# eriq-augustine/KB2E

Measured on AMD Instinct MI355X. Metric: training triples/sec (1/2/4/8 MI355X) + FB15k Hits@10(Filter), higher is better.
Workload: dtype f64

## Files before the change

kb2e_amd/csrc/engine.hip:

```cpp
#include <hip/hip_runtime.h>
#include <hip/hip_ext.h>
#include <hipcub/hipcub.hpp>

#include <algorithm>
#include <cmath>
#include <cstdio>
#include <cstring>
#include <map>
#include <memory>
#include <stdexcept>
#include <string>
#include <vector>

#include "../../include/kb2e_engine.h"
#include "glibc_rand.hpp"
#include "hip_util.hpp"
#include "eval.hpp"
#include "predict.hpp"
#include "host_data.hpp"
#include "kernels_common.hpp"
#include "kernels_index.hpp"
#include "kernels_transe.hpp"
#include "kernels_transe_long.hpp"
#include "kernels_relowner.hpp"
#include "kernels_sampler.hpp"
#include "kernels_parallel.hpp"
#include "kernels_transr_parallel.hpp"
#include "kernels_transr_mfma.hpp"
#include "transr_cons.hpp"
#include "kernels_transh_parallel.hpp"
#include "textio.hpp"

using namespace kb2e;

namespace {

constexpr int kGlibcBlock = 4096;

int bits_for(int64_t v) {
    int b = 1;
    while ((1ll << b) <= v) ++b;
    return b;
}

struct Timer {
    double ms = 0;
    int64_t launches = 0;
};

}

struct kb2e_ctx;
struct MergeState;
void merge_free(MergeState* m);
namespace {
void setup_relowner_buffers(kb2e_ctx* c);
template <typename T>
void run_batch_relowner(kb2e_ctx* c, int64_t b);
void check_dataflow(kb2e_ctx* c);
void build_owner_index(kb2e_ctx* c);
void prepare_relowner_kernels();
void setup_transr_parallel(kb2e_ctx* c);
void build_transr_tiles(kb2e_ctx* c, bool tiles, hipStream_t st, int set);
template <typename T>
void run_batch_transr_parallel(kb2e_ctx* c, int64_t b);
template <typename T, int CH>
void run_batch_transh_parallel(kb2e_ctx* c, int64_t b);
}

struct kb2e_ctx {
    int64_t device_bytes = 0;
    kb2e_config cfg{};
    std::string err;
    GlibcRand rng{1};
    TripleStore ts;
    DevBuf rel_order;
    bool have_triples = false, have_params = false;
    int tables_read = 0;
    int n = 0, ld = 0, ch = 1, nw = 2, esize = 8;
    int64_t B = 0, nb = 0, S = 0;
    int32_t sub = 1;
    int64_t Bs = 0, nbi = 0;
    DevBuf snap_ent, snap_rel, snap_w;
    DevBuf sb_x, sb_d, sb_y, sb_wpart, sb_rpart, sb_pflag, sb_cons_tile, sb_cpairs, sb_vio, sb_cnrows;
    hipStream_t suba_stream = nullptr;
    hipEvent_t ev_adone[2] = {nullptr, nullptr}, ev_bdone[2] = {nullptr, nullptr};
    uint64_t wait_ticks = 0;
    hipStream_t stream = nullptr;

    DevBuf ent, rel, w;
    int64_t w_elems = 0;
    DevBuf heads, tails, rels;
    DevBuf si_[2], sj_[2], side_[2];
    int cur = 0;
    int32_t* pin_si = nullptr;
    int32_t* pin_sj = nullptr;
    uint8_t* pin_side = nullptr;
    hipStream_t side_stream = nullptr;
    DevBuf words, levels, jfin, sidefin, filter_slots, filter_bloom, pr_dev, consumed_dev;
    DevBuf trip;
    int32_t trip_eb = 0, trip_rb = 0;
    DevBuf glibc_pow;
    DevBuf chain_table, chain_super, chain_sc, chain_ch, chain_overflow;
    bool sampler_doubling = false;
    int64_t* pin_consumed = nullptr;
    uint32_t* pin_win = nullptr;
    DevBuf raw_words, glibc_starts, glibc_table, win_dev;
    int64_t nraw = 0, nraw_cap = 0;
    int levels_cap = 0;
    double words_per_sample = 6.0;
    bool prefetch_valid = false;
    uint64_t rng_version = 0, prefetch_version = 0;
    int64_t prefetch_gen = 0, committed_gen = -1, index_pre_gen = -2;
    bool next_pending = false;
    hipEvent_t ev_index = nullptr;
    hipEvent_t ev_sampled = nullptr, ev_epoch_done = nullptr;
    bool host_sampler = false;
    std::vector<int32_t> rp_si, rp_sj;
    std::vector<uint8_t> rp_side;
    int64_t rp_pos = 0;
    KeyLayout kl{};
    int slots = 6;
    DevBuf keys, keys_sorted, sort_tmp, flags, idx, seg_start, nseg, nvalid, batch_seg;
    size_t sort_tmp_bytes = 0, scan_tmp_bytes = 0;
    DevBuf act, loss;
    DevBuf xbits, xreal;
    DevBuf aux, aux2;
    RelOwnerPlan plan;
    DevBuf owner, tickets, ent_done, wsnap, transr_work, transr_work_alt, owner_seg, dataflow_err, wtouched, desc, cdesc, ocount;
    int num_cus = 256;
    uint32_t batch_stamp = 0;
    uint32_t rpar_ptab_mask = 0;
    int32_t gram_min = 48;
    int32_t long_min = 192;
    int32_t apply_long_min = 256;
    int32_t par_long_cap = 1, apply_grid = 256;
    DevBuf par_long_list, par_long_count;
    DevBuf hpar_orth;
    DevBuf hpar_ids;
    DevBuf hpar_tag;
    uint32_t hpar_stamp = 0;
    DevBuf hpar_clk;
    DevBuf hpar_count;
    uint32_t hpar_orth_min = 0;
    int32_t hpar_orth_q = 0;
    DevBuf ev_iota, ev_slot_sorted, ev_inv, seg_row, ev_meta, ev_words;
    int32_t rpar_St = 8, rpar_max_tiles = 1, rpar_tile_threads = 256, rpar_tgroup = 1;
    bool rpar_no_constraint = false;
    bool rpar_mfma = false;
    bool rpar_cons_wave = false;
    size_t rpar_cons_lds = 0;
    bool rpar_cons_seq = false;
    size_t rpar_seq_lds = 0;
    DevBuf rpar_vio;
    bool rpar_cons_wide = false;
    size_t rpar_wide_lds = 0;
    bool rpar_cons_gen = false;
    size_t rpar_gen_lds = 0;
    bool rpar_widep = false;
    WideGeom rpar_wg;
    DevBuf rpar_wsc;
    DevBuf rpar_pflag, rpar_cons_tile, rpar_cpairs, rpar_cnrows;
    DevBuf rpar_y, rpar_wpart, rpar_rpart, rpar_tile_act, rpar_pair, rpar_relpair, rpar_relpair_stamp, rpar_scan_pre, rpar_tiles,
        rpar_ntiles, rpar_tile_first, rpar_rel_begin, rpar_scan;
    DevBuf rpar_ptab;
    DevBuf rpar_batch_t0, rpar_td_r, rpar_td_cnt, rpar_td_kk, rpar_td_ent;
    DevBuf sh_rpar_batch_t0, sh_rpar_td_r, sh_rpar_td_cnt, sh_rpar_td_kk, sh_rpar_td_ent;
    DevBuf rpar_brel, sh_rpar_brel, rpar_bnrel, sh_rpar_bnrel;
    int64_t rpar_brel_cap = 0;
    int32_t* pin_bnrel = nullptr;
    int32_t* pin_sh_bnrel = nullptr;
    hipStream_t fold_stream = nullptr;
    hipEvent_t ev_fold_a = nullptr, ev_fold_b = nullptr;
    DevBuf long_list, long_count;
    DevBuf sh_keys, sh_keys_sorted, sh_sort_tmp, sh_flags, sh_idx, sh_seg_start, sh_nseg, sh_nvalid, sh_batch_seg,
        sh_ev_slot_sorted, sh_ev_inv, sh_seg_row, sh_rpar_ntiles, sh_rpar_rel_begin, sh_rpar_tile_first,
        sh_rpar_tiles, sh_par_long_list, sh_par_long_count;
    DevBuf stats;
    double acc_loss = 0;
    int64_t acc_active = 0;
    int64_t reduced_upto = 0;
    int64_t epoch_pos = 0;
    bool epoch_ready = false;
    bool prof = false;
    int32_t prof_period = 1;
    int64_t prof_counter = 0;
    bool prof_batch = true;
    std::map<std::string, Timer> timers;
    struct Pending {
        std::string name;
        hipEvent_t a, b;
    };
    std::vector<Pending> pending;
    std::vector<hipEvent_t> event_pool;
    MergeState* mg = nullptr;

    ~kb2e_ctx() {
        if (mg) merge_free(mg);
        if (pin_si) (void)hipHostFree(pin_si);
        if (pin_sj) (void)hipHostFree(pin_sj);
        if (pin_side) (void)hipHostFree(pin_side);
        if (pin_win) (void)hipHostFree(pin_win);
        if (pin_consumed) (void)hipHostFree(pin_consumed);
        if (pin_bnrel) (void)hipHostFree(pin_bnrel);
        if (pin_sh_bnrel) (void)hipHostFree(pin_sh_bnrel);
        flush_timers();
        if (ev_sampled) (void)hipEventDestroy(ev_sampled);
        if (ev_epoch_done) (void)hipEventDestroy(ev_epoch_done);
        if (ev_index) (void)hipEventDestroy(ev_index);
        if (side_stream) (void)hipStreamDestroy(side_stream);
        if (suba_stream) (void)hipStreamDestroy(suba_stream);
        for (hipEvent_t e : {ev_adone[0], ev_adone[1], ev_bdone[0], ev_bdone[1]})
            if (e) (void)hipEventDestroy(e);
        if (fold_stream) (void)hipStreamDestroy(fold_stream);
        if (ev_fold_a) (void)hipEventDestroy(ev_fold_a);
        if (ev_fold_b) (void)hipEventDestroy(ev_fold_b);
        for (auto e : event_pool) (void)hipEventDestroy(e);
        if (stream) (void)hipStreamDestroy(stream);
    }

    bool f64() const { return cfg.precision == 64; }
    bool parallel() const { return cfg.schedule == KB2E_SCHEDULE_PARALLEL; }
    int32_t* si() const { return si_[cur].as<int32_t>(); }
    int32_t* sj() const { return sj_[cur].as<int32_t>(); }
    uint8_t* side() const { return side_[cur].as<uint8_t>(); }

    hipEvent_t get_event() {
        if (!event_pool.empty()) {
            hipEvent_t e = event_pool.back();
            event_pool.pop_back();
            return e;
        }
        hipEvent_t e;
        HIPCHK(hipEventCreate(&e));
        return e;
    }

    template <class F>
    void timed(const char* name, F&& f) {
        timed_on(stream, name, f);
    }
    hipEvent_t begin_span() {
        if (!prof || !prof_batch) return nullptr;
        hipEvent_t a = get_event();
        HIPCHK(hipEventRecord(a, stream));
        return a;
    }
    void end_span(const char* name, hipEvent_t a) {
        if (!a) return;
        hipEvent_t b = get_event();
        HIPCHK(hipEventRecord(b, stream));
        pending.push_back({name, a, b});
    }
    template <class F>
    void timed_on(hipStream_t st, const char* name, F&& f) {
        if (!prof || !prof_batch) {
            f();
            return;
        }
        hipEvent_t a = get_event(), b = get_event();
        HIPCHK(hipEventRecord(a, st));
        f();
        HIPCHK(hipEventRecord(b, st));
        pending.push_back({name, a, b});
        if (pending.size() > 4096) flush_timers();
    }

    hipEvent_t span_a = nullptr;
    const char* span_name = nullptr;
    void ev_begin(const char* name, hipEvent_t& a) {
        a = nullptr;
        if (!prof || !prof_batch) return;
        a = span_a = get_event();
        span_name = name;
    }
    void ev_end(hipEvent_t& b) {
        b = nullptr;
        if (!span_a) return;
        b = get_event();
        pending.push_back({span_name, span_a, b});
        span_a = nullptr;
    }
    template <typename... KArgs, typename... Args>
    void launch(void (*kernel)(KArgs...), dim3 grid, dim3 block, size_t lds, hipEvent_t a, hipEvent_t b,
                Args... args) {
        if (a || b) hipExtLaunchKernelGGL(kernel, grid, block, lds, stream, a, b, 0, args...);
        else hipLaunchKernelGGL(kernel, grid, block, lds, stream, args...);
        HIPCHK(hipGetLastError());
    }

    void flush_timers() {
        if (pending.empty()) return;
        (void)hipStreamSynchronize(stream);
        for (auto& p : pending) {
            float ms = 0;
            if (hipEventElapsedTime(&ms, p.a, p.b) == hipSuccess) {
                timers[p.name].ms += ms;
                timers[p.name].launches += 1;
            }
            event_pool.push_back(p.a);
            event_pool.push_back(p.b);
        }
        pending.clear();
    }
};

namespace {

kb2e_status fail(kb2e_ctx* c, kb2e_status s, const std::string& msg) {
    if (c) c->err = msg;
    return s;
}

struct TallyScope {
    int64_t* prev;
    explicit TallyScope(int64_t* t) : prev(DevBuf::tally_now) { DevBuf::tally_now = t; }
    ~TallyScope() { DevBuf::tally_now = prev; }
};

template <class F>
kb2e_status guarded(kb2e_ctx* c, F&& f) {
    if (!c) return KB2E_EINVAL;
    TallyScope ts(&c->device_bytes);
    try {
        return f();
    } catch (const HipError& e) {
        return fail(c, KB2E_EDEVICE, e.what());
    } catch (const Unsupported& e) {
        return fail(c, KB2E_EUNSUPPORTED, e.what());
    } catch (const std::invalid_argument& e) {
        return fail(c, KB2E_EINVAL, e.what());
    } catch (const std::bad_alloc&) {
        return fail(c, KB2E_ENOMEM, "host out of memory");
    } catch (const std::exception& e) {
        return fail(c, KB2E_EDEVICE, e.what());
    }
}


template <typename T>
void upload_rows(kb2e_ctx* c, DevBuf& dst, const double* src, int64_t rows, int n, int ld) {
    std::vector<T> tmp((size_t)rows * ld, T(0));
    for (int64_t r = 0; r < rows; ++r)
        for (int i = 0; i < n; ++i) tmp[(size_t)r * ld + i] = (T)src[(size_t)r * n + i];
    HIPCHK(hipMemcpyAsync(dst.p, tmp.data(), tmp.size() * sizeof(T), hipMemcpyHostToDevice, c->stream));
    HIPCHK(hipStreamSynchronize(c->stream));
}

template <typename T>
void download_rows(kb2e_ctx* c, const DevBuf& src, double* dst, int64_t rows, int n, int ld) {
    std::vector<T> tmp((size_t)rows * ld);
    HIPCHK(hipMemcpyAsync(tmp.data(), src.p, tmp.size() * sizeof(T), hipMemcpyDeviceToHost, c->stream));
    HIPCHK(hipStreamSynchronize(c->stream));
    for (int64_t r = 0; r < rows; ++r)
        for (int i = 0; i < n; ++i) dst[(size_t)r * n + i] = (double)tmp[(size_t)r * ld + i];
}

int64_t w_rows(const kb2e_ctx* c) {
    if (c->cfg.model == KB2E_TRANSH) return c->cfg.num_relations;
    if (c->cfg.model == KB2E_TRANSR) return (int64_t)c->cfg.num_relations * c->n;
    return 0;
}

void sync_wsnap(kb2e_ctx* c) {
    if (c->cfg.model != KB2E_TRANSR) return;
    HIPCHK(hipMemcpyAsync(c->wsnap.p, c->w.p, c->w.bytes, hipMemcpyDeviceToDevice, c->stream));
    HIPCHK(hipStreamSynchronize(c->stream));
}

void upload_tables(kb2e_ctx* c, const double* e, const double* r, const double* w) {
    const int64_t ne = c->cfg.num_entities, nr = c->cfg.num_relations;
    if (c->f64()) {
        if (e) upload_rows<double>(c, c->ent, e, ne, c->n, c->ld);
        if (r) upload_rows<double>(c, c->rel, r, nr, c->n, c->ld);
        if (w && w_rows(c)) upload_rows<double>(c, c->w, w, w_rows(c), c->n, c->ld);
    } else {
        if (e) upload_rows<float>(c, c->ent, e, ne, c->n, c->ld);
        if (r) upload_rows<float>(c, c->rel, r, nr, c->n, c->ld);
        if (w && w_rows(c)) upload_rows<float>(c, c->w, w, w_rows(c), c->n, c->ld);
    }
    if (w) sync_wsnap(c);
}


std::vector<std::pair<DevBuf*, DevBuf*>> index_bufs(kb2e_ctx* c) {
    return {{&c->keys, &c->sh_keys}, {&c->keys_sorted, &c->sh_keys_sorted}, {&c->sort_tmp, &c->sh_sort_tmp},
            {&c->flags, &c->sh_flags}, {&c->idx, &c->sh_idx}, {&c->seg_start, &c->sh_seg_start},
            {&c->nseg, &c->sh_nseg}, {&c->nvalid, &c->sh_nvalid}, {&c->batch_seg, &c->sh_batch_seg},
            {&c->ev_slot_sorted, &c->sh_ev_slot_sorted}, {&c->ev_inv, &c->sh_ev_inv}, {&c->seg_row, &c->sh_seg_row},
            {&c->rpar_ntiles, &c->sh_rpar_ntiles}, {&c->rpar_rel_begin, &c->sh_rpar_rel_begin},
            {&c->rpar_tile_first, &c->sh_rpar_tile_first}, {&c->rpar_tiles, &c->sh_rpar_tiles},
            {&c->rpar_batch_t0, &c->sh_rpar_batch_t0}, {&c->rpar_td_r, &c->sh_rpar_td_r},
            {&c->rpar_td_cnt, &c->sh_rpar_td_cnt}, {&c->rpar_td_kk, &c->sh_rpar_td_kk},
            {&c->rpar_td_ent, &c->sh_rpar_td_ent}, {&c->rpar_brel, &c->sh_rpar_brel},
            {&c->rpar_bnrel, &c->sh_rpar_bnrel},

            {&c->par_long_list, &c->sh_par_long_list}, {&c->par_long_count, &c->sh_par_long_count}};
}

void swap_index(kb2e_ctx* c) {
    for (auto& pr : index_bufs(c)) {
        std::swap(pr.first->p, pr.second->p);
        std::swap(pr.first->bytes, pr.second->bytes);
    }
    std::swap(c->pin_bnrel, c->pin_sh_bnrel);
}

void alloc_shadow_index(kb2e_ctx* c) {
    for (auto& pr : index_bufs(c)) {
        pr.second->free();
        if (pr.first->p) pr.second->alloc(pr.first->bytes);
    }
    c->index_pre_gen = -2;
}

void build_index(kb2e_ctx* c, hipStream_t st, int set) {
    const int64_t nkeys = c->S * c->slots;
    KeyArgs ka{};
    ka.heads = c->heads.as<int32_t>();
    ka.tails = c->tails.as<int32_t>();
    ka.rels = c->rels.as<int32_t>();
    ka.si = c->si_[set].as<int32_t>();
    ka.sj = c->sj_[set].as<int32_t>();
    ka.side = c->side_[set].as<uint8_t>();
    ka.owner = c->cfg.model == KB2E_TRANSE ? nullptr : c->owner.as<int32_t>();
    ka.nsamples = c->S;
    ka.B = (int32_t)c->B;
    ka.sub = c->sub;
    ka.Bs = (int32_t)c->Bs;
    ka.ne = c->cfg.num_entities;
    ka.kl = c->kl;
    ka.keys = c->keys.as<uint64_t>();
    const int grid = (int)((c->S + 255) / 256);
    auto build = [&] {
        if (c->cfg.model == KB2E_TRANSR)
            emit_keys_kernel<8, true><<<grid, 256, 0, st>>>(ka);
        else
            emit_keys_kernel<6, false><<<grid, 256, 0, st>>>(ka);
        HIPCHK(hipGetLastError());
        const int lo_bit = getenv("KB2E_SORT_FULLKEY") ? 0 : c->kl.row_shift();
        size_t tb = c->sort_tmp_bytes;
        if (c->parallel() && c->cfg.model != KB2E_TRANSR) {
            HIPCHK(hipcub::DeviceRadixSort::SortPairs(c->sort_tmp.p, tb, c->keys.as<uint64_t>(),
                                                      c->keys_sorted.as<uint64_t>(), c->ev_iota.as<int32_t>(),
                                                      c->ev_slot_sorted.as<int32_t>(), (int)nkeys, lo_bit,
                                                      c->kl.total_bits(), st));
            inverse_perm_kernel<<<(int)((nkeys + 255) / 256), 256, 0, st>>>(c->ev_slot_sorted.as<int32_t>(),
                                                                                  nkeys, c->ev_inv.as<int32_t>());
            HIPCHK(hipGetLastError());
        } else {
            HIPCHK(hipcub::DeviceRadixSort::SortKeys(c->sort_tmp.p, tb, c->keys.as<uint64_t>(),
                                                     c->keys_sorted.as<uint64_t>(), (int)nkeys, lo_bit,
                                                     c->kl.total_bits(), st));
        }
        const int g2 = (int)((nkeys + 255) / 256);
        seg_flags_kernel<<<g2, 256, 0, st>>>(c->keys_sorted.as<uint64_t>(), nkeys, c->kl,
                                                     c->flags.as<int32_t>(), c->nvalid.as<int32_t>());
        HIPCHK(hipGetLastError());
        tb = c->sort_tmp_bytes;
        HIPCHK(hipcub::DeviceScan::ExclusiveSum(c->sort_tmp.p, tb, c->flags.as<int32_t>(),
                                                c->idx.as<int32_t>(), (int)nkeys, st));
        seg_scatter_kernel<<<g2, 256, 0, st>>>(c->flags.as<int32_t>(), c->idx.as<int32_t>(), nkeys,
                                                       c->seg_start.as<int32_t>(), c->nseg.as<int32_t>(),
                                                       c->nvalid.as<int32_t>());
        HIPCHK(hipGetLastError());
        batch_begin_kernel<<<256, 256, 0, st>>>(c->keys_sorted.as<uint64_t>(), c->seg_start.as<int32_t>(),
                                                        c->nseg.as<int32_t>(), (int)c->nbi, c->kl,
                                                        c->batch_seg.as<int32_t>());
// ... 1439 lines not shown
```

kb2e_amd/csrc/engine_transr_parallel.inc:

```
namespace {

constexpr int32_t kRParLongMin = 128;

template <typename T, bool P, bool G>
const void* tile_fn(int nb) {
    switch (nb) {
        case 1: return (const void*)transr_tile_mfma_kernel<T, P, G, 1>;
        case 2: return (const void*)transr_tile_mfma_kernel<T, P, G, 2>;
        case 3: return (const void*)transr_tile_mfma_kernel<T, P, G, 3>;
        case 4: return (const void*)transr_tile_mfma_kernel<T, P, G, 4>;
        case 5: return (const void*)transr_tile_mfma_kernel<T, P, G, 5>;
        case 6: return (const void*)transr_tile_mfma_kernel<T, P, G, 6>;
        case 7: return (const void*)transr_tile_mfma_kernel<T, P, G, 7>;
        case 8: return (const void*)transr_tile_mfma_kernel<T, P, G, 8>;
    }
    throw std::runtime_error("TransR tile kernel: n > 128");
}

template <typename T>
const void* cons_tile_fn(int nb) {
    switch (nb) {
        case 1: return (const void*)transr_cons_tile_kernel<T, 1>;
        case 2: return (const void*)transr_cons_tile_kernel<T, 2>;
        case 3: return (const void*)transr_cons_tile_kernel<T, 3>;
        case 4: return (const void*)transr_cons_tile_kernel<T, 4>;
        case 5: return (const void*)transr_cons_tile_kernel<T, 5>;
        case 6: return (const void*)transr_cons_tile_kernel<T, 6>;
        case 7: return (const void*)transr_cons_tile_kernel<T, 7>;
        case 8: return (const void*)transr_cons_tile_kernel<T, 8>;
    }
    throw std::runtime_error("transRNorm tile kernel: n > 128");
}

template <typename T>
size_t rpar_lds(const kb2e_ctx* c) {
    return rpar_tile_lds<T>(c->n, c->ld, c->rpar_St);
}

template <typename T>
size_t rmfma_lds(const kb2e_ctx* c, bool cons) {
    return cons ? rmfma_cons_lds<T>(c->n, c->rpar_St) : rmfma_tile_lds<T>(c->n, c->rpar_St);
}

size_t rpar_scan_lds(const kb2e_ctx* c) {
    return (size_t)kScanChunk * 2 * c->n * 8 + (size_t)std::max(1, 1024 / (2 * c->n)) * 2 * c->n * 8;
}

int choose_mfma_samples(int n, int esize, bool tile_only = false) {
    const char* tk = getenv("KB2E_RPAR_TILE_KB");
    const size_t tile_kb = tk ? (size_t)std::max(16, std::min(160, atoi(tk))) : 96;
    for (int St = 8; St >= 1; St >>= 1) {
        const size_t a = esize == 8 ? rmfma_tile_lds<double>(n, St) : rmfma_tile_lds<float>(n, St);
        const size_t b = tile_only ? 0 : esize == 8 ? rmfma_cons_lds<double>(n, St) : rmfma_cons_lds<float>(n, St);
        if (std::max(a, b) <= (tile_only ? tile_kb : 150) * 1024) return St;
    }
    return 0;
}

int choose_tile_samples(int n, int ld, int esize) {
    const size_t budget = (size_t)n * ld * esize > 40 * 1024 ? 150 * 1024 : 64 * 1024;
    for (int St = 32; St > 1; St >>= 1) {
        const size_t b = esize == 8 ? rpar_tile_lds<double>(n, ld, St) : rpar_tile_lds<float>(n, ld, St);
        if (b <= budget) return St;
    }
    return 1;
}

void setup_transr_parallel(kb2e_ctx* c) {
    const kb2e_config& g = c->cfg;
    const size_t es = (size_t)c->esize;
    const char* ck0 = getenv("KB2E_RPAR_CONS");
    const bool wide_planned = c->f64() && c->n > 64 && cons_chainw_supported(c->n) &&
                              !(ck0 && (std::string(ck0) == "jacobi" || std::string(ck0) == "tile"));
    c->rpar_widep = wide_par_supported(c->n);
    const int mst = c->rpar_widep ? 0 : choose_mfma_samples(c->n, c->esize, wide_planned);
    const char* mf = getenv("KB2E_RPAR_MFMA");
    c->rpar_mfma = mst > 0 && !(mf && mf[0] == '0');
    if (c->rpar_widep) c->rpar_wg = wide_setup(c->n, c->ld, c->esize);
    c->rpar_St = c->rpar_widep ? c->rpar_wg.St : c->rpar_mfma ? mst : choose_tile_samples(c->n, c->ld, c->esize);
    if (const char* nc = getenv("KB2E_RPAR_NOC")) c->rpar_no_constraint = nc[0] == '1';
    c->rpar_tile_threads = wide_planned && c->rpar_mfma ? 512 : 256;
    if (const char* tt = getenv("KB2E_RPAR_TILE_THREADS")) c->rpar_tile_threads = atoi(tt) >= 512 ? 512 : 256;
    c->rpar_tgroup = c->rpar_tile_threads == 512 ? 8 : 1;
    if (const char* tg = getenv("KB2E_RPAR_TGROUP")) c->rpar_tgroup = std::max(1, std::min(kTileGroupMax, atoi(tg)));
    if (const char* st = getenv("KB2E_RPAR_ST")) c->rpar_St = std::max(1, std::min(c->rpar_St, atoi(st)));
    if (c->rpar_mfma && 4 * c->rpar_St + 1 > 64) throw std::runtime_error("transRNorm tile: St > 15");
    c->rpar_max_tiles = (int)(std::min<int64_t>(g.num_relations, c->B) + c->B / c->rpar_St + 1);
    const int64_t nkeys = c->S * c->slots;
    c->rpar_y.alloc((size_t)c->B * 2 * c->ld * es);
    const bool cw = cons_wave_supported(c->n) && mst > 0;
    c->rpar_wpart.alloc((size_t)c->rpar_max_tiles * (cw ? kConsPpt : 1) * c->n * c->ld * es);
    c->rpar_rpart.alloc((size_t)c->rpar_max_tiles * c->ld * es);
    c->rpar_tile_act.alloc((size_t)(nkeys + 1) * 4);
    c->rpar_pair.alloc((size_t)c->B * 4 * c->ld * es);
    c->rpar_relpair.alloc((size_t)g.num_relations * c->ld * es);
    c->rpar_relpair_stamp.alloc((size_t)g.num_relations * 4);
    memset_sync(c->rpar_relpair_stamp.p, 0, c->rpar_relpair_stamp.bytes);
    c->rpar_tiles.alloc((size_t)(nkeys + 1) * sizeof(RTile));
    c->rpar_ntiles.alloc((size_t)(nkeys + 1) * 4);
    c->rpar_tile_first.alloc((size_t)(nkeys + 1) * 4);
    c->rpar_rel_begin.alloc((size_t)c->nbi * 4);
    c->rpar_brel_cap = std::min<int64_t>(g.num_relations, c->Bs);
    c->rpar_brel.alloc((size_t)c->nbi * c->rpar_brel_cap * 4);
    c->rpar_bnrel.alloc((size_t)c->nbi * 4);
    for (int32_t** h : {&c->pin_bnrel, &c->pin_sh_bnrel}) {
        if (*h) (void)hipHostFree(*h);
        *h = nullptr;
        HIPCHK(hipHostMalloc((void**)h, (size_t)c->nbi * 4, 0));
        std::memset(*h, 0, (size_t)c->nbi * 4);
    }
    if (c->rpar_widep) c->rpar_wsc.alloc((size_t)c->rpar_brel_cap * c->n * c->ld * 8);
    else c->rpar_wsc.free();
    if (c->sub > 1) {
        c->snap_ent.alloc(c->ent.bytes);
        c->snap_rel.alloc(c->rel.bytes);
        c->snap_w.alloc(c->w.bytes);
        for (DevBuf* d : {&c->snap_ent, &c->snap_rel, &c->snap_w}) memset_sync(d->p, 0, d->bytes);
        if (!c->suba_stream) {
            int lo = 0, hi = 0;
            HIPCHK(hipDeviceGetStreamPriorityRange(&lo, &hi));
            HIPCHK(hipStreamCreateWithPriority(&c->suba_stream, hipStreamNonBlocking, hi));
            for (hipEvent_t* e : {&c->ev_adone[0], &c->ev_adone[1], &c->ev_bdone[0], &c->ev_bdone[1]})
                HIPCHK(hipEventCreateWithFlags(e, hipEventDisableTiming));
        }
    } else {
        for (DevBuf* d : {&c->snap_ent, &c->snap_rel, &c->snap_w}) d->free();
    }
    if (g.num_entities >= (1 << kPtabEntBits) - 1 || g.num_relations >= (1 << kPtabRelBits) - 1 ||
        c->B * 4 >= (1 << kPtabSlotBits))
        throw std::invalid_argument("PARALLEL TransR: at most 2^24 - 2 entities, 2^18 - 2 relations, 2^20 - 1 samples a batch");
    {
        size_t sz = 1024;
        while (sz < (size_t)c->B * 4 * 3) sz <<= 1;
        c->rpar_ptab_mask = (uint32_t)(sz - 1);
        c->rpar_ptab.alloc(3 * sz * 8);
        memset_sync(c->rpar_ptab.p, 0xff, 3 * sz * 8);
    }
    const int scan_chunk = c->rpar_widep ? c->rpar_wg.chunk : kScanChunk;
    c->rpar_scan.alloc((size_t)((2 * c->B + scan_chunk - 1) / scan_chunk) * 2 * c->n * 8);
    c->rpar_scan_pre.alloc(c->rpar_scan.bytes);
    c->rpar_pflag.alloc((size_t)c->B * 4);
    c->rpar_cons_tile.alloc((size_t)c->rpar_max_tiles * (cw ? kConsPpt : 1) * 4);
    if (cw) {
        c->rpar_cpairs.alloc((size_t)c->rpar_max_tiles * 2 * kCPairs * 4);
        c->rpar_vio.alloc((size_t)c->rpar_max_tiles * kCPairs * 4);
        c->rpar_cnrows.alloc((size_t)c->rpar_max_tiles * 4);
    }
    size_t tb = 0;
    HIPCHK(hipcub::DeviceScan::ExclusiveSum(nullptr, tb, (int32_t*)nullptr, (int32_t*)nullptr, (int)(nkeys + 1),
                                            c->stream));
    if (tb > c->sort_tmp_bytes) {
        c->sort_tmp_bytes = tb;
        c->sort_tmp.alloc(tb);
    }
    const size_t lds = c->f64() ? rpar_lds<double>(c) : rpar_lds<float>(c);
    auto allow = [&](const void* k) {
        (void)hipFuncSetAttribute(k, hipFuncAttributeMaxDynamicSharedMemorySize, (int)lds);
    };
    allow((const void*)transr_tile_kernel<double, true, true>);
    allow((const void*)transr_tile_kernel<double, true, false>);
    allow((const void*)transr_tile_kernel<double, false, true>);
    allow((const void*)transr_tile_kernel<float, true, true>);
    allow((const void*)transr_tile_kernel<float, true, false>);
    allow((const void*)transr_tile_kernel<float, false, true>);
    allow((const void*)transr_constraint_kernel<double>);
    allow((const void*)transr_constraint_kernel<float>);
    c->rpar_cons_wave = false;
    if (c->rpar_mfma) {
        const size_t l1 = c->f64() ? rmfma_lds<double>(c, false) : rmfma_lds<float>(c, false);
        const size_t l2 = c->f64() ? rmfma_lds<double>(c, true) : rmfma_lds<float>(c, true);
        const int nb = rm_np(c->n) / 16;
        for (const void* k : {tile_fn<double, true, true>(nb), tile_fn<double, true, false>(nb),
                              tile_fn<double, false, true>(nb), tile_fn<float, true, true>(nb),
                              tile_fn<float, true, false>(nb), tile_fn<float, false, true>(nb)})
            (void)hipFuncSetAttribute(k, hipFuncAttributeMaxDynamicSharedMemorySize, (int)l1);
        if (!wide_planned)
            for (int nb = 1; nb <= 8; ++nb)
                (void)hipFuncSetAttribute(c->f64() ? cons_tile_fn<double>(nb) : cons_tile_fn<float>(nb),
                                          hipFuncAttributeMaxDynamicSharedMemorySize, (int)l2);
        const char* ck = getenv("KB2E_RPAR_CONS");
        c->rpar_cons_wave = cw && c->rpar_St <= 8 && !(ck && std::string(ck) == "tile");
        if (c->rpar_cons_wave) c->rpar_cons_lds = cons_wave_setup(c->n, c->rpar_St, c->esize);
        c->rpar_cons_seq = c->rpar_cons_wave && c->f64() && !(ck && std::string(ck) == "jacobi");
        if (c->rpar_cons_seq) {
            c->rpar_seq_lds = cons_seq_setup(c->n);
        }
    }
    {
        const char* ck = getenv("KB2E_RPAR_CONS");
        const bool jac = ck && (std::string(ck) == "jacobi" || std::string(ck) == "tile");
        const char* chn = getenv("KB2E_RPAR_CHAIN");
        c->rpar_cons_wide = !c->rpar_cons_seq && c->f64() && cons_chainw_supported(c->n) && !jac;
        if (c->rpar_cons_wide) c->rpar_wide_lds = cons_chainw_setup(c->n);
        const bool force_gen = chn && std::string(chn) == "gen";
        if (force_gen && !jac) c->rpar_cons_seq = c->rpar_cons_wide = false;
        c->rpar_cons_gen = !c->rpar_cons_seq && !c->rpar_cons_wide && !jac && cons_chaing_supported(c->n);
        if (c->rpar_cons_gen) c->rpar_gen_lds = cons_chaing_setup(c->n, c->esize);
        if (c->rpar_widep) c->rpar_cons_seq = c->rpar_cons_wide = c->rpar_cons_gen = false;
        if (!c->rpar_cons_seq && !c->rpar_cons_wide && !c->rpar_cons_gen && !c->rpar_widep && !c->rpar_no_constraint &&
            !jac)
            throw Unsupported("PARALLEL TransR: no pair-by-pair transRNorm at this width");
    }
    if (c->rpar_cons_wave || c->rpar_mfma) {
        const size_t nt = (size_t)c->nbi * c->rpar_max_tiles + 1;
        c->rpar_batch_t0.alloc((size_t)(c->nbi + 1) * 4);
        c->rpar_td_r.alloc(nt * 4);
        c->rpar_td_cnt.alloc(nt * 4);
        c->rpar_td_kk.alloc(nt * 8 * 4);
        c->rpar_td_ent.alloc(nt * 32 * 4);
    } else {
        for (DevBuf* d : {&c->rpar_batch_t0, &c->rpar_td_r, &c->rpar_td_cnt, &c->rpar_td_kk, &c->rpar_td_ent}) d->free();
    }
    {
        const std::pair<DevBuf*, DevBuf*> sets[] = {
            {&c->sb_x, &c->xreal}, {&c->sb_d, &c->aux}, {&c->sb_y, &c->rpar_y}, {&c->sb_wpart, &c->rpar_wpart},
            {&c->sb_rpart, &c->rpar_rpart}, {&c->sb_pflag, &c->rpar_pflag}, {&c->sb_cons_tile, &c->rpar_cons_tile},
            {&c->sb_cpairs, &c->rpar_cpairs}, {&c->sb_vio, &c->rpar_vio}, {&c->sb_cnrows, &c->rpar_cnrows}};
        for (const auto& pr : sets) {
            pr.first->free();
            if (c->sub > 1 && pr.second->p) {
                pr.first->alloc(pr.second->bytes);
                memset_sync(pr.first->p, 0, pr.first->bytes);
            }
        }
    }
    for (const void* k : {(const void*)rpar_scan_energy_kernel<double>, (const void*)rpar_scan_energy_kernel<float>})
        (void)hipFuncSetAttribute(k, hipFuncAttributeMaxDynamicSharedMemorySize, (int)rpar_scan_lds(c));
    (void)hipGetLastError();
}

void build_transr_tiles(kb2e_ctx* c, bool tiles, hipStream_t st, int set) {
    const int64_t nkeys = c->S * c->slots;
    rtile_count_kernel<<<1024, 256, 0, st>>>(c->keys_sorted.as<uint64_t>(), c->seg_start.as<int32_t>(),
                                                    c->nseg.as<int32_t>(), nkeys + 1, c->kl, c->cfg.num_entities,
                                                    c->rpar_St, c->rpar_ntiles.as<int32_t>(),
                                                    c->rpar_rel_begin.as<int32_t>());
    HIPCHK(hipGetLastError());
    if (!tiles) return;
    size_t tb = c->sort_tmp_bytes;
    HIPCHK(hipcub::DeviceScan::ExclusiveSum(c->sort_tmp.p, tb, c->rpar_ntiles.as<int32_t>(),
                                            c->rpar_tile_first.as<int32_t>(), (int)(nkeys + 1), st));
    rtile_scatter_kernel<<<1024, 256, 0, st>>>(c->rpar_ntiles.as<int32_t>(), c->rpar_tile_first.as<int32_t>(),
                                                      c->nseg.as<int32_t>(), c->rpar_tiles.as<RTile>());
    HIPCHK(hipGetLastError());
    if (c->rpar_brel.p) {
        rel_list_kernel<<<(int)c->nbi, 1024, 0, st>>>(c->rpar_rel_begin.as<int32_t>(), c->batch_seg.as<int32_t>(),
                                                     c->seg_row.as<int32_t>(), c->cfg.num_entities,
                                                     c->rel_order.as<int32_t>(), c->cfg.num_relations,
                                                     c->rpar_brel_cap, c->rpar_brel.as<int32_t>(),
                                                     c->rpar_bnrel.as<int32_t>());
        HIPCHK(hipGetLastError());
        HIPCHK(hipMemcpyAsync(c->pin_bnrel, c->rpar_bnrel.p, (size_t)c->nbi * 4, hipMemcpyDeviceToHost, st));
    }
    if (c->rpar_td_r.p) {
        RTileDescArgs d{};
        d.keys = c->keys_sorted.as<uint64_t>();
        d.seg_start = c->seg_start.as<int32_t>();
        d.seg_row = c->seg_row.as<int32_t>();
        d.tiles = c->rpar_tiles.as<RTile>();
        d.tile_first = c->rpar_tile_first.as<int32_t>();
        d.nseg = c->nseg.as<int32_t>();
        d.batch_seg = c->batch_seg.as<int32_t>();
        d.nb = (int32_t)c->nbi;
        d.sub = c->sub;
        d.Bs = (int32_t)c->Bs;
        d.St = c->rpar_St;
        d.ne = c->cfg.num_entities;
        d.B = (int32_t)c->B;
        d.kl = c->kl;
        d.si = c->si_[set].as<int32_t>();
        d.sj = c->sj_[set].as<int32_t>();
        d.side = c->side_[set].as<uint8_t>();
        d.heads = c->heads.as<int32_t>();
        d.tails = c->tails.as<int32_t>();
        d.batch_t0 = c->rpar_batch_t0.as<int32_t>();
        d.td_r = c->rpar_td_r.as<int32_t>();
        d.td_cnt = c->rpar_td_cnt.as<int32_t>();
        d.td_kk = c->rpar_td_kk.as<int32_t>();
        d.td_ent = c->rpar_td_ent.as<int32_t>();
        rtile_desc_kernel<<<2048, 256, 0, st>>>(d);
        HIPCHK(hipGetLastError());
    }
}

DevBuf& buf_set(int set, DevBuf& s0, DevBuf& s1) { return set ? s1 : s0; }

bool sub_overlap_on() {
    const char* e = getenv("KB2E_SUB_OVERLAP");
    return !(e && e[0] == '0');
}

template <typename T>
void run_subbatch_transr_parallel(kb2e_ctx* c, int64_t b, int j) {
    const bool ov = c->sub > 1 && sub_overlap_on();
    const bool side = ov && j > 0;
    const int set = ov ? (j & 1) : 0;
    hipStream_t sa = side ? c->suba_stream : c->stream;
    const int64_t ib = b * c->sub + j;
    const int64_t first = b * c->B + (int64_t)j * c->Bs;
    const int64_t cnt = std::min<int64_t>(c->Bs, c->B - (int64_t)j * c->Bs);
    RParArgs a{};
    a.heads = c->heads.as<int32_t>();
    a.tails = c->tails.as<int32_t>();
    a.rels = c->rels.as<int32_t>();
    a.si = c->si() + first;
    a.sj = c->sj() + first;
    a.side = c->side() + first;
    a.B = (int32_t)cnt;
    a.n = c->n;
    a.ld = c->ld;
    a.ne = c->cfg.num_entities;
    a.nr = c->cfg.num_relations;
    a.St = c->rpar_St;
    a.tgroup = c->rpar_tgroup;
    a.batch = (int32_t)ib;
    a.lr = c->cfg.learning_rate;
    a.margin = c->cfg.margin;
    a.compat = c->cfg.transr_compat;
    a.l1 = c->cfg.distance == 0;
    a.keys = c->keys_sorted.as<uint64_t>();
    a.seg_start = c->seg_start.as<int32_t>();
    a.batch_seg = c->batch_seg.as<int32_t>();
    a.seg_row = c->seg_row.as<int32_t>();
    a.rel_begin = c->rpar_rel_begin.as<int32_t>();
    a.tile_first = c->rpar_tile_first.as<int32_t>();
    a.tiles = c->rpar_tiles.as<RTile>();
    a.kl = c->kl;
    a.act = c->act.as<uint8_t>() + first;
    a.loss = c->loss.as<double>() + first;
    a.proj = c->aux2.as<double>();
    a.tile_act = c->rpar_tile_act.as<int32_t>();
    a.batch_t0 = c->rpar_batch_t0.as<int32_t>();
    a.td_r = c->rpar_td_r.as<int32_t>();
    a.td_cnt = c->rpar_td_cnt.as<int32_t>();
    a.td_kk = c->rpar_td_kk.as<int32_t>();
    a.td_ent = c->rpar_td_ent.as<int32_t>();
    a.brel = c->rpar_brel.as<int32_t>() + ib * c->rpar_brel_cap;
    a.nrel = c->pin_bnrel[ib];
    if (a.nrel < 1 || a.nrel > c->rpar_brel_cap) throw std::logic_error("batch relation count out of range");
    {
        unsigned long long* t0 = c->rpar_ptab.as<unsigned long long>();
        const size_t sz = (size_t)c->rpar_ptab_mask + 1;
        a.ptab = t0 + (c->batch_stamp % 3) * sz;
        a.ptab_next = t0 + ((c->batch_stamp + 1) % 3) * sz;
        a.ptab_mask = c->rpar_ptab_mask;
    }
    RParBufs<T> bf{};
    bf.ent = c->ent.as<T>();
    bf.rel = c->rel.as<T>();
    bf.W = c->w.as<T>();
    bf.x = buf_set(set, c->xreal, c->sb_x).as<T>();
    bf.d = buf_set(set, c->aux, c->sb_d).as<T>();
    bf.y = buf_set(set, c->rpar_y, c->sb_y).as<T>();
    bf.wpart = buf_set(set, c->rpar_wpart, c->sb_wpart).as<T>();
    bf.rpart = buf_set(set, c->rpar_rpart, c->sb_rpart).as<T>();
    bf.pair = c->rpar_pair.as<T>();
    bf.relpair = c->rpar_relpair.as<T>();
    bf.relpair_stamp = c->rpar_relpair_stamp.as<uint32_t>();
    bf.stamp = ++c->batch_stamp;
    bf.err = c->dataflow_err.as<uint32_t>() + 1;
    if (c->rpar_mfma) {
        bf.pflag = buf_set(set, c->rpar_pflag, c->sb_pflag).as<uint8_t>();
        bf.cons_tile = buf_set(set, c->rpar_cons_tile, c->sb_cons_tile).as<int32_t>();
        bf.cons_ppt = c->rpar_cons_wave ? kConsPpt : 1;
        bf.cpairs = buf_set(set, c->rpar_cpairs, c->sb_cpairs).as<int32_t>();
        bf.vio = buf_set(set, c->rpar_vio, c->sb_vio).as<int32_t>();
        bf.cnrows = buf_set(set, c->rpar_cnrows, c->sb_cnrows).as<int32_t>();
        bf.stats = getenv("KB2E_RPAR_STATS") != nullptr;
        bf.last_renorm = c->rpar_cons_seq ? 1 : 0;
        if (const char* dbg = getenv("KB2E_CONS_DBG")) bf.dbg = atoi(dbg);
        if (const char* cl = getenv("KB2E_RPAR_CHAIN_LIST")) bf.chain_list = std::max(64, atoi(cl));
        if (const char* ct = getenv("KB2E_RPAR_CHAIN_TILES")) bf.chain_tiles = std::max(1, atoi(ct));
        if (const char* rc = getenv("KB2E_RPAR_REC_CAP")) bf.rec_cap = std::max(4, atoi(rc));
    }
    if (c->rpar_cons_wide || c->rpar_cons_gen || c->rpar_widep) {
        bf.pflag = buf_set(set, c->rpar_pflag, c->sb_pflag).as<uint8_t>();
        if (const char* dbg = getenv("KB2E_CONS_DBG")) bf.dbg = atoi(dbg);
        bf.stats = getenv("KB2E_RPAR_STATS") != nullptr;
        bf.last_renorm = 1;
    }
    RParBufs<T> bfa = bf;
    if (c->sub > 1) {
        bfa.ent = c->snap_ent.as<T>();
        bfa.rel = c->snap_rel.as<T>();
        bfa.W = c->snap_w.as<T>();
    }
    if (side && j == 1) HIPCHK(hipStreamWaitEvent(sa, c->ev_adone[0], 0));
    if (side && j >= 2) HIPCHK(hipStreamWaitEvent(sa, c->ev_bdone[set], 0));
    auto a_done = [&] {
        if (!ov) return;
        HIPCHK(hipEventRecord(c->ev_adone[set], sa));
        if (side) HIPCHK(hipStreamWaitEvent(c->stream, c->ev_adone[set], 0));
    };
    auto b_done = [&] {
        if (ov) HIPCHK(hipEventRecord(c->ev_bdone[set], c->stream));
    };
    if (c->rpar_widep) {
        c->timed_on(sa, "score", [&] {
            wide_phase_a<T>(a, bfa, c->rpar_wg, c->rpar_max_tiles, c->rpar_scan.as<double>(),
                            c->rpar_scan_pre.as<double>(), c->transr_work.as<double>(),
                            c->transr_work_alt.as<double>(), sa);
        });
        if (c->cfg.transr_compat) std::swap(c->transr_work.p, c->transr_work_alt.p);
        a_done();
        c->timed("apply", [&] {
            wide_phase_b<T>(a, bf, c->rpar_wg, c->rpar_wsc.as<double>(), !c->rpar_no_constraint,
                            (int)std::min<int64_t>(c->cfg.num_relations, c->Bs), c->stream);
        });
        b_done();
        if (c->pending.size() > 4096) c->flush_timers();
        return;
    }
    const size_t lds = rpar_lds<T>(c);
    const int tgrid = c->rpar_max_tiles;
    const int rel_waves = (int)std::min<int64_t>(c->cfg.num_relations, c->B) * (c->n + 1);
    const int rgrid = (rel_waves + 3) / 4;
    const int egrid = 256;
    const bool mf = c->rpar_mfma;
    const size_t lt = mf ? rmfma_lds<T>(c, false) : lds;
    const size_t lc = mf ? rmfma_lds<T>(c, true) : lds;
    const int tb = mf ? c->rpar_tile_threads : 256;
    auto tile = [&](auto proj, auto grad) {
        constexpr bool P = decltype(proj)::value, G = decltype(grad)::value;
        if (mf) {
            void* args[] = {&a, &bfa};
            int pt = tb;
            if (P && !G) {
                pt = 256;
                if (const char* e = getenv("KB2E_RPAR_PROJ_THREADS")) pt = atoi(e) >= 512 ? 512 : 256;
            }
            HIPCHK(hipLaunchKernel(tile_fn<T, P, G>(rm_np(c->n) / 16), dim3(tgrid), dim3(pt), args,
                                   rmfma_tile_lds<T>(c->n, c->rpar_St, P, G), sa));
        } else {
            transr_tile_kernel<T, P, G><<<tgrid, tb, lt, sa>>>(a, bfa);
        }
        HIPCHK(hipGetLastError());
    };
    using yes = std::true_type;
    using no = std::false_type;
    auto pair_first = [&] {
        if (c->rpar_no_constraint) return;
        transr_pair_first_kernel<<<(int)((4 * c->B + 255) / 256), 256, 0, sa>>>(a);
        HIPCHK(hipGetLastError());
    };
    c->timed_on(sa, "score", [&] {
        if (c->cfg.transr_compat) {
            if (c->rpar_cons_wave) proj_wave_launch<T>(a, bfa, tgrid, sa);
            else tile(yes(), no());
            const int64_t calls = 2 * (int64_t)a.B;
            const int nchunks = (int)((calls + kScanChunk - 1) / kScanChunk);
            rpar_scan_sums_kernel<<<nchunks, 256, 0, sa>>>(a.proj, calls, c->ld, c->n,
                                                                  c->rpar_scan.as<double>());
            const char* sp = getenv("KB2E_RPAR_SCAN_PREFIX");
            const bool use_pre = sp ? sp[0] == '1' : nchunks > kScanDirectMax;
            double* pre = nullptr;
            if (use_pre) {
                pre = c->rpar_scan_pre.as<double>();
                rpar_scan_prefix_kernel<<<(2 * c->n + 31) / 32, 1024, 0, sa>>>(
                    c->rpar_scan.as<double>(), nchunks, 2 * c->n, c->transr_work.as<double>(), pre);
            }
            rpar_scan_energy_kernel<T><<<nchunks, 1024, rpar_scan_lds(c), sa>>>(
                a, bfa, c->rpar_scan.as<double>(), nchunks, c->transr_work.as<double>(),
                c->transr_work_alt.as<double>(), pre);
            HIPCHK(hipGetLastError());
            std::swap(c->transr_work.p, c->transr_work_alt.p);
            if (c->rpar_cons_wave) grad_wave_launch<T>(a, bfa, tgrid, sa);
            else tile(no(), yes());
        } else if (c->rpar_cons_wave) {
            proj_wave_launch<T>(a, bfa, tgrid, sa);
            grad_wave_launch<T>(a, bfa, tgrid, sa);
        } else {
            tile(yes(), yes());
            pair_first();
        }
    });
    a_done();
    hipEvent_t e0, e1;
    c->ev_begin("apply", e0);
    const char* fz = getenv("KB2E_RPAR_FUSE");
    const bool fuse = !(fz && fz[0] == '0');
    const char* r8 = getenv("KB2E_RPAR_ROWS8");
    const int rmode = c->n <= 64 ? 4 : (c->n <= 128 && r8 && r8[0] == '1') ? 8 : 0;
    const bool rows4 = rmode != 0;
    const int rel_waves4 = (int)std::min<int64_t>(c->cfg.num_relations, c->B) * ((c->n + 4) / 4);
    const int rw = rows4 ? rel_waves4 : rel_waves;
    const int fgrid = egrid + (rw + 15) / 16;
    auto rows_fn = [&](auto pass1) {
        constexpr bool P = decltype(pass1)::value;
        return rmode == 4 ? transr_rows_kernel<T, P, 4> : rmode == 8 ? transr_rows_kernel<T, P, 8>
                                                                     : transr_rows_kernel<T, P, 0>;
    };
    using yes1 = std::true_type;
    if (c->rpar_no_constraint) {
        c->ev_end(e1);
        c->launch(rows_fn(yes1()), dim3(fgrid), dim3(1024), 0, e0, e1, a, bf, kRParLongMin, egrid);
        b_done();
        return;
    }
    if (fuse) {
        c->launch(rows_fn(yes1()), dim3(fgrid), dim3(1024), 0, e0, nullptr, a, bf, kRParLongMin, egrid);
    } else {
        c->launch(transr_rel_rows_kernel<T, true>, dim3(rgrid), dim3(256), 0, e0, nullptr, a, bf);
        transr_entity_kernel<T, true><<<egrid, 1024, 0, c->stream>>>(a, bf, kRParLongMin);
        HIPCHK(hipGetLastError());
    }
    if (mf && c->rpar_cons_seq) {
        if constexpr (std::is_same<T, double>::value) cons_seq_launch(a, bf, c->rpar_seq_lds, c->stream);
    } else if (c->rpar_cons_gen) {
        cons_chaing_launch<T>(a, bf, c->rpar_gen_lds, c->stream);
    } else if (c->rpar_cons_wide) {
        if constexpr (std::is_same<T, double>::value) cons_chainw_launch(a, bf, c->rpar_wide_lds, c->stream);
    } else if (mf && c->rpar_cons_wave) {
        cons_wave_launch<T>(a, bf, tgrid, c->rpar_cons_lds, c->stream);
    } else if (mf) {
        void* args[] = {&a, &bf};
        HIPCHK(hipLaunchKernel(cons_tile_fn<T>(rm_np(c->n) / 16), dim3(tgrid), dim3(512), args, lc, c->stream));
    } else {
        transr_constraint_kernel<T><<<tgrid, 256, lc, c->stream>>>(a, bf);
    }
    HIPCHK(hipGetLastError());
    c->ev_end(e1);
    const char* f2 = getenv("KB2E_RPAR_FUSE2");
    if (c->rpar_cons_seq || c->rpar_cons_wide || c->rpar_cons_gen) {
        c->launch(transr_entity_kernel<T, false>, dim3(egrid), dim3(1024), 0, nullptr, e1, a, bf, kRParLongMin);
    } else if (f2 && f2[0] == '1') {
        c->launch(rows_fn(std::false_type()), dim3(fgrid), dim3(1024), 0, nullptr, e1, a, bf, kRParLongMin, egrid);
    } else {
        if (rmode == 4) transr_rel_rows4_kernel<T, false, 4><<<(rel_waves4 + 3) / 4, 256, 0, c->stream>>>(a, bf);
        else if (rmode == 8) transr_rel_rows4_kernel<T, false, 8><<<(rel_waves4 + 3) / 4, 256, 0, c->stream>>>(a, bf);
        else transr_rel_rows_kernel<T, false><<<rgrid, 256, 0, c->stream>>>(a, bf);
        HIPCHK(hipGetLastError());
        c->launch(transr_entity_kernel<T, false>, dim3(egrid), dim3(1024), 0, nullptr, e1, a, bf, kRParLongMin);
    }
    b_done();
    if (c->pending.size() > 4096) c->flush_timers();
}

template <typename T>
void run_batch_transr_parallel(kb2e_ctx* c, int64_t b) {
    if (c->sub > 1) {
        for (auto pr : {std::make_pair(&c->snap_ent, &c->ent), std::make_pair(&c->snap_rel, &c->rel),
                        std::make_pair(&c->snap_w, &c->w)})
            HIPCHK(hipMemcpyAsync(pr.first->p, pr.second->p, pr.second->bytes, hipMemcpyDeviceToDevice, c->stream));
    }
    for (int j = 0; j < c->sub; ++j) run_subbatch_transr_parallel<T>(c, b, j);
}

}
```

kb2e_amd/csrc/kernels_transr_parallel.hpp:

```cpp
#pragma once

#include <type_traits>

#include "kernels_common.hpp"

namespace kb2e {

struct RTile {
    int32_t seg, q;
};

struct RParArgs {
    const int32_t* heads;
    const int32_t* tails;
    const int32_t* rels;
    const int32_t* si;
    const int32_t* sj;
    const uint8_t* side;
    int32_t B, n, ld, ne, nr, St;
    int32_t batch;
    int32_t tgroup;
    double lr, margin;
    int32_t compat, l1;
    const uint64_t* keys;
    const int32_t* seg_start;
    const int32_t* batch_seg;
    const int32_t* seg_row;
    const int32_t* rel_begin;
    const int32_t* tile_first;
    const RTile* tiles;
    KeyLayout kl;
    uint8_t* act;
    double* loss;
    double* proj;
    int32_t* tile_act;
    unsigned long long* ptab;
    unsigned long long* ptab_next;
    uint32_t ptab_mask;
    const int32_t* batch_t0;
    const int32_t* td_r;
    const int32_t* td_cnt;
    const int32_t* td_kk;
    const int32_t* td_ent;
    const int32_t* brel;
    int32_t nrel;
};

static __attribute__((unused)) __global__ __launch_bounds__(1024) void rel_list_kernel(
    const int32_t* rel_begin, const int32_t* batch_seg, const int32_t* seg_row, int32_t ne, const int32_t* rel_order,
    int32_t nr, int64_t cap, int32_t* brel, int32_t* nrel) {
    __shared__ int32_t wsum[16];
    const int b = blockIdx.x, t = threadIdx.x, w = t >> 6, l = t & 63;
    const int s0 = rel_begin[b], s1 = batch_seg[b + 1];
    int32_t* out = brel + (int64_t)b * cap;
    int total = 0;
    for (int base = 0; base < nr; base += 1024) {
        const int q = base + t;
        const int r = q < nr ? rel_order[q] : -1;
        bool here = false;
        if (r >= 0 && s0 < s1) {
            int lo = s0, hi = s1 - 1;
            const int want = ne + r;
            while (lo < hi) {
                const int mid = (lo + hi) >> 1;
                if (seg_row[mid] < want) lo = mid + 1;
                else hi = mid;
            }
            here = seg_row[lo] == want;
        }
        const uint64_t m = __ballot(here);
        if (l == 0) wsum[w] = __popcll(m);
        __syncthreads();
        int off = total;
        for (int k = 0; k < w; ++k) off += wsum[k];
        int all = 0;
        for (int k = 0; k < 16; ++k) all += wsum[k];
        if (here) out[off + __popcll(m & ((1ull << l) - 1))] = r;
        total += all;
        __syncthreads();
    }
    if (t == 0) nrel[b] = total;
}

constexpr int kPtabEntBits = 24, kPtabRelBits = 18, kPtabSlotBits = 22;
constexpr unsigned long long kPtabEmpty = ~0ull;

__device__ __forceinline__ unsigned long long ptab_key(int r, int e) {
    return ((unsigned long long)r << kPtabEntBits) | (unsigned long long)e;
}
__device__ __forceinline__ uint32_t ptab_hash(int r, int e) {
    return ((uint32_t)e * 2654435761u) ^ ((uint32_t)r * 0x9E3779B1u + 0x7F4A7C15u);
}

__device__ __forceinline__ void ptab_insert(const RParArgs& a, int r, int e, int slot) {
    const unsigned long long key = ptab_key(r, e);
    const unsigned long long word = (key << kPtabSlotBits) | (unsigned long long)slot;
    uint32_t h = ptab_hash(r, e) & a.ptab_mask;
    while (true) {
        const unsigned long long old = atomicCAS(a.ptab + h, kPtabEmpty, word);
        if (old == kPtabEmpty) return;
        if ((old >> kPtabSlotBits) == key) {
            atomicMin(a.ptab + h, word);
            return;
        }
        h = (h + 1) & a.ptab_mask;
    }
}

__device__ __forceinline__ int ptab_first(const RParArgs& a, int r, int e) {
    const unsigned long long key = ptab_key(r, e);
    uint32_t h = ptab_hash(r, e) & a.ptab_mask;
    while (true) {
        const unsigned long long w = a.ptab[h];
        if (w == kPtabEmpty) return -1;
        if ((w >> kPtabSlotBits) == key) return (int)(w & ((1ull << kPtabSlotBits) - 1));
        h = (h + 1) & a.ptab_mask;
    }
}

__device__ __forceinline__ void ptab_clear_next(const RParArgs& a, int64_t tid, int64_t nthreads) {
    for (int64_t q = tid; q <= (int64_t)a.ptab_mask; q += nthreads) a.ptab_next[q] = kPtabEmpty;
}

__device__ __forceinline__ bool transr_pair_dup(const RParArgs& a, int slot, int r, int e) {
    return ptab_first(a, r, e) < slot;
}
__device__ __forceinline__ bool transr_relpair_dup(const RParArgs& a, int r) {
    return ptab_first(a, r, r) >= 0;
}

static __attribute__((unused)) __global__ __launch_bounds__(256) void transr_pair_first_kernel(RParArgs a) {
    const int slot = blockIdx.x * blockDim.x + threadIdx.x;
    ptab_clear_next(a, slot, (int64_t)gridDim.x * blockDim.x);
    if (slot >= 4 * a.B) return;
    const int kk = slot >> 2, u = (slot >> 1) & 1, role = slot & 1;
    if (!a.act[kk]) return;
    const int i0 = a.si[kk], jj = a.sj[kk];
    const int h = a.heads[i0], tt = a.tails[i0];
    const int hh = u ? (a.side[kk] ? h : jj) : h;
    const int th = u ? (a.side[kk] ? jj : tt) : tt;
    ptab_insert(a, a.rels[i0], role ? th : hh, slot);
}

template <typename T>
struct RParBufs {
    T* ent;
    T* rel;
    T* W;
    T* x;
    T* d;
    T* y;
    T* wpart;
    T* rpart;
    T* pair;
    T* relpair;
    uint32_t* relpair_stamp;
    uint32_t stamp;
    uint8_t* pflag;
    int32_t* cons_tile;
    int32_t cons_ppt;
    int32_t* cpairs;
    int32_t* cnrows;
    int32_t stats;
    int32_t last_renorm;
    int32_t dbg;
    int32_t chain_list;
    int32_t chain_tiles;
    int32_t rec_cap;
    int32_t* vio;
    uint32_t* err;
};

__host__ __device__ constexpr int rm_up16_host_dev(int v) { return (v + 15) & ~15; }
constexpr int kCPairs = 64;

template <typename T>
__host__ __device__ constexpr int rpar_lds_w(int n, int ld) {
    return n * ld;
}

__device__ __forceinline__ void tile_range(const RParArgs& a, int t, int& r, int& e0, int& cnt) {
    const RTile tl = a.tiles[t];
    const int p0 = a.seg_start[tl.seg], p1 = a.seg_start[tl.seg + 1];
    r = a.seg_row[tl.seg] - a.ne;
    const int ns = (p1 - p0) / 2;
    const int f = tl.q * a.St;
    e0 = p0 + 2 * f;
    cnt = min(a.St, ns - f);
}

template <typename T>
__device__ __forceinline__ void stage_matrix(T* Wl, const T* Wg, int n, int ld) {
    for (int idx = threadIdx.x; idx < n * ld; idx += blockDim.x) Wl[idx] = Wg[idx];
}

template <typename T>
__device__ __forceinline__ void project4(const T* Wl, int ld, int n, const T* v4 , T (&p)[4][2]) {
    const int l = lane_id();
    const int i = 2 * l;
#pragma unroll
    for (int q = 0; q < 4; ++q) p[q][0] = p[q][1] = T(0);
    if (i >= n) return;
    for (int j = 0; j < n; ++j) {
        const T w0 = Wl[j * ld + i], w1 = Wl[j * ld + i + 1];
#pragma unroll
        for (int q = 0; q < 4; ++q) {
            const T vj = v4[q * ld + j];
            p[q][0] += w0 * vj;
            p[q][1] += w1 * vj;
        }
    }
}

template <typename T>
__device__ __forceinline__ void matvec_rows(const T* Wl, int ld, int n, const T* xl, T (&y)[2]) {
    const int l = lane_id();
    const int j = 2 * l;
    y[0] = y[1] = T(0);
    if (j >= n) return;
    const T* r0 = Wl + j * ld;
    const T* r1 = Wl + (j + 1) * ld;
    const bool has1 = j + 1 < n;
    for (int i = 0; i < n; ++i) {
        const T xi = xl[i];
        y[0] += r0[i] * xi;
        if (has1) y[1] += r1[i] * xi;
    }
}

template <typename T>
__device__ __forceinline__ void lane_pair_load(const T* row, int n, T (&v)[2]) {
    const int e = 2 * lane_id();
    v[0] = e < n ? row[e] : T(0);
    v[1] = e + 1 < n ? row[e + 1] : T(0);
}
template <typename T>
__device__ __forceinline__ void lane_pair_store(T* row, int n, const T (&v)[2]) {
    const int e = 2 * lane_id();
    if (e < n) row[e] = v[0];
    if (e + 1 < n) row[e + 1] = v[1];
}

template <typename T>
__device__ __forceinline__ void rank_sum_rows(const T* Dl, const T* Xl, int U, int ld, int n, int j, T (&acc)[2]) {
    const int i = 2 * lane_id();
    acc[0] = acc[1] = T(0);
    if (i >= n) return;
    for (int u = 0; u < U; ++u) {
        const T dj = Dl[u * ld + j];
        acc[0] += dj * Xl[u * ld + i];
        acc[1] += dj * Xl[u * ld + i + 1];
    }
}

template <typename T>
__host__ __device__ constexpr size_t rpar_tile_lds(int n, int ld, int St) {
    return sizeof(T) * ((size_t)n * ld + 4 * 4 * (size_t)ld + 2 * (4 * (size_t)St + 1) * ld + 4 * (size_t)St + 1) +
           sizeof(int) * (4 * (size_t)St + 1);
}

template <typename T, bool PROJ, bool GRAD>
__global__ __launch_bounds__(256) void transr_tile_kernel(RParArgs a, RParBufs<T> bf) {
    extern __shared__ __attribute__((aligned(16))) char smem[];
    const int t = a.tile_first[a.batch_seg[a.batch]] + blockIdx.x;
    if (t >= a.tile_first[a.batch_seg[a.batch + 1]]) return;
    int r, e0, cnt;
    tile_range(a, t, r, e0, cnt);
    const int n = a.n, ld = a.ld;
    T* Wl = (T*)smem;
    T* vec = Wl + n * ld;
    T* Xl = vec + 16 * ld;
    T* Dl = Xl + (4 * a.St + 1) * ld;
    T* coef = Dl + (4 * a.St + 1) * ld;
    const int w = threadIdx.x >> 6, l = lane_id();
    stage_matrix(Wl, bf.W + (int64_t)r * n * ld, n, ld);
    __syncthreads();
    T* v4 = vec + w * 4 * ld;
    for (int q = w; q < cnt; q += 4) {
        const int kk = a.kl.kk_of(a.keys[e0 + 2 * q]);
        if (PROJ) {
            const int i0 = a.si[kk], jj = a.sj[kk];
            const int h = a.heads[i0], tt = a.tails[i0];
            const int nh = a.side[kk] ? h : jj, nt = a.side[kk] ? jj : tt;
            T vh[2], vt[2], vnh[2], vnt[2], vr[2];
            lane_pair_load(bf.ent + (int64_t)h * ld, n, vh);
            lane_pair_load(bf.ent + (int64_t)tt * ld, n, vt);
            lane_pair_load(bf.ent + (int64_t)nh * ld, n, vnh);
            lane_pair_load(bf.ent + (int64_t)nt * ld, n, vnt);
            lane_pair_load(bf.rel + (int64_t)r * ld, n, vr);
            lane_pair_store(v4 + 0 * ld, n, vh);
            lane_pair_store(v4 + 1 * ld, n, vt);
            lane_pair_store(v4 + 2 * ld, n, vnh);
            lane_pair_store(v4 + 3 * ld, n, vnt);
            wave_lds_sync();
            T p[4][2];
            project4(Wl, ld, n, v4, p);
            T ep = T(0), en = T(0);
            T xp[2], xn[2];
#pragma unroll
            for (int k = 0; k < 2; ++k) {
                const bool ok = 2 * l + k < n;
                const T dp = p[1][k] - p[0][k] - vr[k];
                const T dn = p[3][k] - p[2][k] - vr[k];
                ep += ok ? (a.l1 ? fabs(dp) : dp * dp) : T(0);
                en += ok ? (a.l1 ? fabs(dn) : dn * dn) : T(0);
                xp[k] = ok ? (a.l1 ? (dp > T(0) ? T(1) : T(-1)) : T(2) * dp) : T(0);
                xn[k] = ok ? (a.l1 ? (dn > T(0) ? T(1) : T(-1)) : T(2) * dn) : T(0);
            }
            const T dpos[2] = {vh[0] - vt[0], vh[1] - vt[1]};
            const T dneg[2] = {vnh[0] - vnt[0], vnh[1] - vnt[1]};
            lane_pair_store(bf.x + ((int64_t)kk * 2 + 0) * ld, n, xp);
            lane_pair_store(bf.x + ((int64_t)kk * 2 + 1) * ld, n, xn);
            lane_pair_store(bf.d + ((int64_t)kk * 2 + 0) * ld, n, dpos);
            lane_pair_store(bf.d + ((int64_t)kk * 2 + 1) * ld, n, dneg);
            if (a.compat) {
                double* pr = a.proj + (int64_t)kk * 4 * ld;
#pragma unroll
                for (int k = 0; k < 2; ++k) {
                    const int e = 2 * l + k;
                    if (e >= n) continue;
                    pr[e] = (double)p[0][k];
                    pr[ld + e] = (double)p[1][k];
                    pr[2 * ld + e] = (double)p[2][k];
                    pr[3 * ld + e] = (double)p[3][k];
                }
            } else {
                ep = wave_sum(ep);
                en = wave_sum(en);
                const bool active = (double)ep + a.margin > (double)en;
                if (l == 0) {
                    a.act[kk] = active ? 1 : 0;
                    a.loss[kk] = active ? a.margin + (double)ep - (double)en : 0.0;
                }
                if (GRAD) {
#pragma unroll
                    for (int u = 0; u < 2; ++u) {
                        const T c = active ? (T)(-(u ? 1.0 : -1.0) * a.lr) : T(0);
                        const T* dv = u ? dneg : dpos;
                        const T dsc[2] = {c * dv[0], c * dv[1]};
                        lane_pair_store(Xl + (2 * q + u) * ld, n, u ? xn : xp);
                        lane_pair_store(Dl + (2 * q + u) * ld, n, dsc);
                        if (l == 0) coef[2 * q + u] = c;
                    }
                }
            }
            wave_lds_sync();
            lane_pair_store(v4 + 0 * ld, n, xp);
            lane_pair_store(v4 + 1 * ld, n, xn);
            wave_lds_sync();
            T yp[2], yn[2];
            matvec_rows(Wl, ld, n, v4 + 0 * ld, yp);
            matvec_rows(Wl, ld, n, v4 + 1 * ld, yn);
            lane_pair_store(bf.y + ((int64_t)kk * 2 + 0) * ld, n, yp);
            lane_pair_store(bf.y + ((int64_t)kk * 2 + 1) * ld, n, yn);
            wave_lds_sync();
        }
    }
    if (!GRAD) return;
    if (!PROJ) {
        for (int q = w; q < cnt; q += 4) {
            const int kk = a.kl.kk_of(a.keys[e0 + 2 * q]);
            const bool act = a.act[kk] != 0;
#pragma unroll
            for (int u = 0; u < 2; ++u) {
                const T c = act ? (T)(-(u ? 1.0 : -1.0) * a.lr) : T(0);
                T xv[2], dv[2];
                lane_pair_load(bf.x + ((int64_t)kk * 2 + u) * ld, n, xv);
                lane_pair_load(bf.d + ((int64_t)kk * 2 + u) * ld, n, dv);
                dv[0] *= c;
                dv[1] *= c;
                lane_pair_store(Xl + (2 * q + u) * ld, n, xv);
                lane_pair_store(Dl + (2 * q + u) * ld, n, dv);
                if (l == 0) coef[2 * q + u] = c;
            }
        }
    }
    __syncthreads();
    const int U = 2 * cnt;
    T* wp = bf.wpart + (int64_t)blockIdx.x * n * ld;
    for (int j = w; j < n; j += 4) {
        T acc[2];
        rank_sum_rows(Dl, Xl, U, ld, n, j, acc);
        lane_pair_store(wp + (int64_t)j * ld, n, acc);
    }
    if (w == 0) {
        T acc[2] = {T(0), T(0)};
        const int i = 2 * l;
        for (int u = 0; u < U; ++u) {
            const T c = coef[u];
            if (i < n) acc[0] += c * Xl[u * ld + i];
            if (i + 1 < n) acc[1] += c * Xl[u * ld + i + 1];
        }
        lane_pair_store(bf.rpart + (int64_t)blockIdx.x * ld, n, acc);
        if (l == 0) {
            int nact = 0;
            for (int u = 0; u < U; ++u) nact += coef[u] != T(0);
            a.tile_act[t] = nact;
        }
    }
}
template <typename T, bool NORM>
__device__ __forceinline__ void transr_rel_rows_wave(RParArgs a, RParBufs<T> bf, int gw) {
    const int rows = a.n + 1;
    const int s = a.rel_begin[a.batch] + gw / rows;
    const int j = gw % rows;
    if (s >= a.batch_seg[a.batch + 1]) return;
    if (!NORM && j == a.n) return;
    const int r = a.seg_row[s] - a.ne;
    const int t0 = a.tile_first[s], t1 = a.tile_first[s + 1];
    const int n = a.n, ld = a.ld;
    const int tb = a.tile_first[a.batch_seg[a.batch]];
    const bool sel = !NORM && bf.cons_tile;
    const int ppt = sel ? bf.cons_ppt : 1;
    const int u0 = sel ? (t0 - tb) * ppt : t0, u1 = sel ? (t1 - tb) * ppt : t1;
    const int ub = sel ? 0 : tb;
    const int32_t* const fl = sel ? bf.cons_tile : a.tile_act;
    auto flags = [fl, u1](int base) {
        const int u = base + lane_id();
        const int f = u < u1 ? fl[u] : 0;
        return (uint64_t)__ballot(f != 0);
    };
    uint64_t any = 0;
    for (int base = u0; base < u1 && !any; base += kWave) any = flags(base);
    if (!any) return;
    T* row = j < n ? bf.W + ((int64_t)r * n + j) * ld : bf.rel + (int64_t)r * ld;
    T v[2];
    lane_pair_load(row, n, v);
    for (int base = u0; base < u1; base += kWave) {
        uint64_t m = (NORM || sel) ? flags(base) : (uint64_t)__ballot(base + lane_id() < u1);
        while (m) {
            T p[8][2];
            bool use[8];
#pragma unroll
            for (int q = 0; q < 8; ++q) {
                use[q] = m != 0;
                const int64_t lt = use[q] ? base + __builtin_ctzll(m) - ub : 0;
                m &= m - 1;
                if (use[q]) lane_pair_load(j < n ? bf.wpart + (lt * n + j) * ld : bf.rpart + lt * ld, n, p[q]);
            }
#pragma unroll
            for (int q = 0; q < 8; ++q)
                if (use[q]) {
                    v[0] += p[q][0];
                    v[1] += p[q][1];
                }
        }
    }
    if (NORM) {
        const T len = sqrt(wave_sum(v[0] * v[0] + v[1] * v[1]));
        v[0] = v[0] / len;
        v[1] = v[1] / len;
    }
    lane_pair_store(row, n, v);
}

template <typename T, bool NORM, int E = 4>
__device__ __forceinline__ void transr_rel_rows4_wave(RParArgs a, RParBufs<T> bf, int gw) {
    using T2 = typename std::conditional<sizeof(T) == 8, double2, float2>::type;
    constexpr int E2 = E / 2, NQ = E == 4 ? 8 : 4;
    const int n = a.n, ld = a.ld;
    const int RW = (n + 4) >> 2;
    const int s = a.rel_begin[a.batch] + gw / RW;
    if (s >= a.batch_seg[a.batch + 1]) return;
    const int l = lane_id(), e0 = E * (l & 15);
    const int j = (gw % RW) * 4 + (l >> 4);
    const bool jok = NORM ? j <= n : j < n;
    const int r = a.seg_row[s] - a.ne;
    const int t0 = a.tile_first[s], t1 = a.tile_first[s + 1];
    const int tb = a.tile_first[a.batch_seg[a.batch]];
    const bool sel = !NORM && bf.cons_tile;
    const int ppt = sel ? bf.cons_ppt : 1;
    const int u0 = sel ? (t0 - tb) * ppt : t0, u1 = sel ? (t1 - tb) * ppt : t1;
    const int ub = sel ? 0 : tb;
    const int32_t* const fl = sel ? bf.cons_tile : a.tile_act;
    auto flags = [fl, u1, l](int base) {
        const int u = base + l;
        return (uint64_t)__ballot(u < u1 && fl[u] != 0);
// ... 93 lines not shown
            const int kk = a.kl.kk_of(a.keys[e0 + 2 * q]);
            if (a.act[kk]) {
                const int i0 = a.si[kk], jj = a.sj[kk];
                const int h = a.heads[i0], tt = a.tails[i0];
                const int hh = u ? (a.side[kk] ? h : jj) : h;
                const int th = u ? (a.side[kk] ? jj : tt) : tt;
                const int e = role ? th : hh;
                if (!transr_pair_dup(a, (kk * 2 + u) * 2 + role, r, e)) ent = e;
            }
        } else if (!transr_relpair_dup(a, r)) {
            ent = r;
        }
        ent_of[pq] = ent;
    }
    stage_matrix(Wl, bf.W + (int64_t)r * n * ld, n, ld);
    __syncthreads();
    T* v4 = vec + w * 4 * ld;
    const int i = 2 * l;
    for (int pq = w; pq < npairs; pq += 4) {
        const int ent = ent_of[pq];
        bool live = ent >= 0;
        for (int k = 0; live && k < pq; ++k) live = ent_of[k] != ent;
        T a0[2] = {T(0), T(0)}, G[2] = {T(0), T(0)}, da[2] = {T(0), T(0)};
        if (live) {
            lane_pair_load(bf.ent + (int64_t)ent * ld, n, a0);
            const T s0 = wave_sum(a0[0] * a0[0] + a0[1] * a0[1]);
            lane_pair_store(v4, n, a0);
            wave_lds_sync();
            T p[2] = {T(0), T(0)};
            if (i < n)
                for (int j = 0; j < n; ++j) {
                    const T aj = v4[j];
                    p[0] += Wl[j * ld + i] * aj;
                    p[1] += Wl[j * ld + i + 1] * aj;
                }
            if (i + 1 >= n) p[1] = T(0);
            if (i >= n) p[0] = T(0);
            wave_lds_sync();
            for (int m = 0; m < kRParMaxIter; ++m) {
                const T xx = wave_sum(p[0] * p[0] + p[1] * p[1]);
                if (!(xx > T(1))) break;
                G[0] += T(2) * p[0];
                G[1] += T(2) * p[1];
                lane_pair_store(v4, n, p);
                wave_lds_sync();
                T v[2];
                matvec_rows(Wl, ld, n, v4, v);
                lane_pair_store(v4 + ld, n, v);
                wave_lds_sync();
                T q[2] = {T(0), T(0)};
                if (i < n)
                    for (int j = 0; j < n; ++j) {
                        const T vj = v4[ld + j];
                        q[0] += Wl[j * ld + i] * vj;
                        q[1] += Wl[j * ld + i + 1] * vj;
                    }
                wave_lds_sync();
                const T c = T(2) * T(a.lr) * s0;
#pragma unroll
                for (int k = 0; k < 2; ++k) p[k] = i + k < n ? p[k] - T(2) * T(a.lr) * q[k] - c * p[k] : T(0);
            }
            lane_pair_store(v4, n, G);
            wave_lds_sync();
            matvec_rows(Wl, ld, n, v4, da);
            da[0] *= T(-a.lr);
            da[1] *= T(-a.lr);
            wave_lds_sync();
        }
        if (pq < 4 * cnt) {
            const int q = pq >> 2, u = (pq >> 1) & 1, role = pq & 1;
            const int kk = a.kl.kk_of(a.keys[e0 + 2 * q]);
            if (a.act[kk]) lane_pair_store(bf.pair + (((int64_t)kk * 2 + u) * 2 + role) * ld, n, da);
        } else {
            lane_pair_store(bf.relpair + (int64_t)r * ld, n, da);
            if (l == 0) bf.relpair_stamp[r] = bf.stamp;
        }
        const T dv[2] = {T(-a.lr) * a0[0], T(-a.lr) * a0[1]};
        lane_pair_store(Xl + pq * ld, n, G);
        lane_pair_store(Dl + pq * ld, n, dv);
    }
    __syncthreads();
    T* wp = bf.wpart + (int64_t)blockIdx.x * n * ld;
    for (int j = w; j < n; j += 4) {
        T acc[2];
        rank_sum_rows(Dl, Xl, npairs, ld, n, j, acc);
        lane_pair_store(wp + (int64_t)j * ld, n, acc);
    }
}

constexpr int kRParWaves = 16;

__device__ __forceinline__ int rpar_entity_last(const RParArgs& a, int p0, int p1, int first, int stride) {
    const int l = lane_id();
    int last = -1;
    for (int base = p0 + first * kWave; base < p1; base += stride * kWave) {
        const int p = base + l;
        if (p < p1) {
            const uint64_t key = a.keys[p];
            const int kk = a.kl.kk_of(key);
            if (a.act[kk] && (key & (kRoleHead | kRoleTail))) last = max(last, kk * 2 + (int)((key >> 3) & 1));
        }
    }
#pragma unroll
    for (int s = 32; s >= 1; s >>= 1) last = max(last, __shfl_xor(last, s));
    return last;
}

template <typename T, bool GRAD>
__device__ __forceinline__ void rpar_entity_events(const RParArgs& a, const RParBufs<T>& bf, int row, int p0, int p1,
                                                   int first, int stride, int last, T (&acc)[2], T (&acc2)[2],
                                                   bool& dirty, bool& dirty2, bool& er_seen) {
    const int n = a.n, ld = a.ld, l = lane_id();
    const bool split = !GRAD && bf.last_renorm;
    for (int base = p0 + first * kWave; base < p1; base += stride * kWave) {
        const int p = base + l;
        int src = -1;
        int src2 = -1;
        T c = T(0);
        bool nrm = false, er = false, post = false;
        if (p < p1) {
            const uint64_t key = a.keys[p];
            const int kk = a.kl.kk_of(key);
            if (a.act[kk]) {
                const int u = (int)((key >> 3) & 1);
                const uint32_t roles = (uint32_t)(key & 7);
                const bool hd = roles & kRoleHead, tl = roles & kRoleTail;
                er = roles & kRoleEntRel;
                if (GRAD) {
                    nrm = hd || tl;
                    if (hd != tl) {
                        src = kk * 2 + u;
                        c = (T)((hd ? -1.0 : 1.0) * (u ? 1.0 : -1.0) * a.lr);
                    }
                } else {
                    const int s0 = (kk * 2 + u) * 2;
                    const bool ph = hd && (!bf.pflag || bf.pflag[s0]);
                    const bool pt = tl && (!bf.pflag || bf.pflag[s0 + 1]);
                    nrm = ph || pt;
                    post = split && kk * 2 + u == last;
                    if (ph) src = s0;
                    if (pt) {
                        if (src < 0) src = s0 + 1;
                        else src2 = s0 + 1;
                    }
                }
            }
        }
        if (__ballot(nrm && !post)) dirty = true;
        if (__ballot(nrm && post)) dirty2 = true;
        if (__ballot(er)) er_seen = true;
        const T* tab = GRAD ? bf.y : bf.pair;
        for (int pass = 0; pass < (GRAD ? 1 : 2); ++pass) {
            const int mine = pass ? src2 : src;
            uint64_t m = __ballot(mine >= 0);
            const uint64_t pm = __ballot(post);
            while (m) {
                int ev[4];
                int k = 0;
                for (; k < 4 && m; ++k) {
                    ev[k] = __builtin_ctzll(m);
                    m &= m - 1;
                }
                T v[4][2];
#pragma unroll
                for (int q = 0; q < 4; ++q)
                    if (q < k) lane_pair_load(tab + (int64_t)readlane_i32(mine, ev[q]) * ld, n, v[q]);
#pragma unroll
                for (int q = 0; q < 4; ++q)
                    if (q < k) {
                        const T cq = GRAD ? readlane_f(c, ev[q]) : T(1);
                        T(&dst)[2] = ((pm >> ev[q]) & 1) ? acc2 : acc;
                        dst[0] += cq * v[q][0];
                        dst[1] += cq * v[q][1];
                    }
            }
        }
    }
}

template <typename T, bool GRAD>
__device__ __forceinline__ void rpar_entity_finish(const RParArgs& a, const RParBufs<T>& bf, int row, T (&acc)[2],
                                                   T (&acc2)[2], bool dirty, bool dirty2, bool er_seen, int last) {
    const int n = a.n, ld = a.ld;
    const bool split = !GRAD && bf.last_renorm;
    if (!GRAD && er_seen && row < a.nr && bf.relpair_stamp[row] == bf.stamp) {
        T dv[2];
        lane_pair_load(bf.relpair + (int64_t)row * ld, n, dv);
        if (split && last < 0) {
            acc2[0] += dv[0];
            acc2[1] += dv[1];
            dirty2 = true;
        } else {
            acc[0] += dv[0];
            acc[1] += dv[1];
            dirty = true;
        }
    }
    if (!dirty && !dirty2) return;
    T* ptr = bf.ent + (int64_t)row * ld;
    T v[2];
    lane_pair_load(ptr, n, v);
    if (dirty) {
        v[0] += acc[0];
        v[1] += acc[1];
    }
    if (GRAD || (split && dirty)) {
        const T len = sqrt(wave_sum(v[0] * v[0] + v[1] * v[1]));
        v[0] = v[0] / len;
        v[1] = v[1] / len;
    }
    if (dirty2) {
        v[0] += acc2[0];
        v[1] += acc2[1];
    }
    lane_pair_store(ptr, n, v);
}

template <typename T, bool GRAD>
__device__ __forceinline__ void transr_entity_block(RParArgs a, RParBufs<T> bf, int32_t long_min, int bid, int G) {
    __shared__ T part[kRParWaves][4][kWave];
    __shared__ int flags[4];
    __shared__ int longs[1024], nlong;
    const int w = threadIdx.x >> 6, l = lane_id();
    const bool split = !GRAD && bf.last_renorm;
    const int s0 = a.batch_seg[a.batch], s1 = a.rel_begin[a.batch];
    const int blockIdx_x = bid;
    for (int c0 = s0 + blockIdx_x; c0 < s1; c0 += G * (int)blockDim.x) {
        if (threadIdx.x == 0) nlong = 0;
        __syncthreads();
        const int cs = c0 + G * (int)threadIdx.x;
        if (cs < s1 && a.seg_start[cs + 1] - a.seg_start[cs] >= long_min) longs[atomicAdd(&nlong, 1)] = cs;
        __syncthreads();
        const int nl = nlong;
        for (int li = 0; li < nl; ++li) {
        const int s = longs[li];
        const int p0 = a.seg_start[s], p1 = a.seg_start[s + 1];
        const int row = a.seg_row[s];
        if (threadIdx.x < 4) flags[threadIdx.x] = threadIdx.x == 3 ? -1 : 0;
        __syncthreads();
        int last = -1;
        if (split) {
            last = rpar_entity_last(a, p0, p1, w, kRParWaves);
            if (l == 0) atomicMax(&flags[3], last);
            __syncthreads();
            last = flags[3];
        }
        T acc[2] = {T(0), T(0)}, acc2[2] = {T(0), T(0)};
        bool dirty = false, dirty2 = false, er = false;
        rpar_entity_events<T, GRAD>(a, bf, row, p0, p1, w, kRParWaves, last, acc, acc2, dirty, dirty2,
                                    er);
        part[w][0][l] = acc[0];
        part[w][1][l] = acc[1];
        part[w][2][l] = acc2[0];
        part[w][3][l] = acc2[1];
        if (l == 0 && dirty) atomicOr(&flags[0], 1);
        if (l == 0 && er) atomicOr(&flags[1], 1);
        if (l == 0 && dirty2) atomicOr(&flags[2], 1);
        __syncthreads();
        if (w == 0) {
            acc[0] = part[0][0][l];
            acc[1] = part[0][1][l];
            acc2[0] = part[0][2][l];
            acc2[1] = part[0][3][l];
            for (int v = 1; v < kRParWaves; ++v) {
                acc[0] += part[v][0][l];
                acc[1] += part[v][1][l];
                acc2[0] += part[v][2][l];
                acc2[1] += part[v][3][l];
            }
            rpar_entity_finish<T, GRAD>(a, bf, row, acc, acc2, flags[0] != 0, flags[2] != 0, flags[1] != 0, last);
        }
        __syncthreads();
        }
    }
    for (int s = s0 + blockIdx_x * kRParWaves + w; s < s1; s += G * kRParWaves) {
        const int p0 = a.seg_start[s], p1 = a.seg_start[s + 1];
        if (p1 - p0 >= long_min) continue;
        const int row = a.seg_row[s];
        const int last = split ? rpar_entity_last(a, p0, p1, 0, 1) : -1;
        T acc[2] = {T(0), T(0)}, acc2[2] = {T(0), T(0)};
        bool dirty = false, dirty2 = false, er = false;
        rpar_entity_events<T, GRAD>(a, bf, row, p0, p1, 0, 1, last, acc, acc2, dirty, dirty2, er);
        rpar_entity_finish<T, GRAD>(a, bf, row, acc, acc2, dirty, dirty2, er, last);
    }
}

template <typename T, bool GRAD>
__global__ __launch_bounds__(1024) void transr_entity_kernel(RParArgs a, RParBufs<T> bf, int32_t long_min) {
    transr_entity_block<T, GRAD>(a, bf, long_min, blockIdx.x, gridDim.x);
}

template <typename T, bool PASS1, int RM>
__global__ __launch_bounds__(1024) void transr_rows_kernel(RParArgs a, RParBufs<T> bf, int32_t long_min,
                                                           int32_t egrid) {
    const int gw = (((int)blockIdx.x - egrid) * (int)blockDim.x + (int)threadIdx.x) >> 6;
    if ((int)blockIdx.x < egrid) transr_entity_block<T, PASS1>(a, bf, long_min, blockIdx.x, egrid);
    else if (RM == 4) transr_rel_rows4_wave<T, PASS1, 4>(a, bf, gw);
    else if (RM == 8) transr_rel_rows4_wave<T, PASS1, 8>(a, bf, gw);
    else transr_rel_rows_wave<T, PASS1>(a, bf, gw);
}

constexpr int kScanChunk = 64;

static __attribute__((unused)) __global__ __launch_bounds__(256) void rpar_scan_sums_kernel(const double* proj, int64_t calls, int32_t ld,
                                                             int32_t n, double* sums) {
    const int c = blockIdx.x;
    const int64_t c0 = (int64_t)c * kScanChunk, c1 = min<int64_t>(calls, c0 + kScanChunk);
    for (int e = threadIdx.x; e < 2 * n; e += blockDim.x) {
        const int side = e / n, i = e % n;
        double s[4] = {0, 0, 0, 0};
        for (int64_t k = c0; k < c1; k += 16) {
            double v[16];
#pragma unroll
            for (int q = 0; q < 16; ++q) v[q] = k + q < c1 ? proj[((k + q) * 2 + side) * ld + i] : 0.0;
#pragma unroll
            for (int q = 0; q < 16; ++q) s[q & 3] += v[q];
        }
        sums[(int64_t)c * 2 * n + e] = (s[0] + s[1]) + (s[2] + s[3]);
    }
}

constexpr int kScanDirectMax = 256;

static __attribute__((unused)) __global__ __launch_bounds__(1024) void rpar_scan_prefix_kernel(
    const double* sums, int32_t nchunks, int32_t E2, const double* work_in, double* pre) {
    __shared__ double tot[32][33];
    const int el = threadIdx.x & 31, part = threadIdx.x >> 5;
    const int e = blockIdx.x * 32 + el;
    const int per = (nchunks + 31) / 32;
    const int c0 = part * per, c1 = min(nchunks, c0 + per);
    double s = 0.0;
    if (e < E2) {
        for (int c = c0; c < c1; c += 8) {
            double v[8];
#pragma unroll
            for (int q = 0; q < 8; ++q) v[q] = c + q < c1 ? sums[(int64_t)(c + q) * E2 + e] : 0.0;
#pragma unroll
            for (int q = 0; q < 8; ++q) s += v[q];
        }
    }
    tot[part][el] = s;
    __syncthreads();
    double run = e < E2 ? work_in[e] : 0.0;
    for (int p = 0; p < part; ++p) run += tot[p][el];
    if (e >= E2) return;
    for (int c = c0; c < c1; c += 8) {
        double v[8];
#pragma unroll
        for (int q = 0; q < 8; ++q) v[q] = c + q < c1 ? sums[(int64_t)(c + q) * E2 + e] : 0.0;
#pragma unroll
        for (int q = 0; q < 8; ++q)
            if (c + q < c1) {
                pre[(int64_t)(c + q) * E2 + e] = run;
                run += v[q];
            }
    }
}

template <typename T>
__global__ __launch_bounds__(1024) void rpar_scan_energy_kernel(RParArgs a, RParBufs<T> bf, const double* sums,
                                                                int32_t nchunks, const double* work_in,
                                                                double* work_out, const double* pre) {
    extern __shared__ __attribute__((aligned(16))) char smem[];
    double* run_l = (double*)smem;
    const int c = blockIdx.x, n = a.n, ld = a.ld;
    const int64_t calls = 2 * (int64_t)a.B;
    const int64_t c0 = (int64_t)c * kScanChunk, c1 = min<int64_t>(calls, c0 + kScanChunk);
    __shared__ int act_l[kScanChunk / 2];
    const int nsamp = (int)(c1 - c0) / 2;
    int pent = -1, prel = -1;
    if ((int)threadIdx.x < 4 * nsamp) {
        const int64_t kk = c0 / 2 + (threadIdx.x >> 2);
        const int u = (threadIdx.x >> 1) & 1, role = threadIdx.x & 1;
        const int i0 = a.si[kk], jj = a.sj[kk];
        const int h = a.heads[i0], tt = a.tails[i0];
        const int hh = u ? (a.side[kk] ? h : jj) : h;
        const int th = u ? (a.side[kk] ? jj : tt) : tt;
        pent = role ? th : hh;
        prel = a.rels[i0];
    }
    const int E2 = 2 * n, G = max(1, (int)blockDim.x / E2);
    double* part = run_l + kScanChunk * E2;
    if (!pre && (int)threadIdx.x < G * E2) {
        const int g = threadIdx.x / E2, e = threadIdx.x % E2;
        double s[4] = {0, 0, 0, 0};
        for (int q0 = g * 16; q0 < c; q0 += G * 16) {
            double v[16];
#pragma unroll
            for (int q = 0; q < 16; ++q) v[q] = q0 + q < c ? sums[(int64_t)(q0 + q) * E2 + e] : 0.0;
#pragma unroll
            for (int q = 0; q < 16; ++q) s[q & 3] += v[q];
        }
        part[g * E2 + e] = (s[0] + s[1]) + (s[2] + s[3]);
    }
    __syncthreads();
    for (int e = threadIdx.x; e < 2 * n; e += blockDim.x) {
        double run;
        if (pre) {
            run = pre[(int64_t)c * E2 + e];
        } else {
            double p = 0.0;
            for (int g = 0; g < G; ++g) p += part[g * E2 + e];
            run = work_in[e] + p;
        }
        const int side = e / n, i = e % n;
        for (int64_t k = c0; k < c1; k += 16) {
            double v[16];
#pragma unroll
            for (int q = 0; q < 16; ++q) v[q] = k + q < c1 ? a.proj[((k + q) * 2 + side) * ld + i] : 0.0;
#pragma unroll
            for (int q = 0; q < 16; ++q)
                if (k + q < c1) {
                    run += v[q];
                    run_l[(k + q - c0) * 2 * n + e] = run;
                }
        }
        if (c == nchunks - 1) work_out[e] = run;
    }
    __syncthreads();
    const int w = threadIdx.x >> 6, nw = blockDim.x >> 6, l = lane_id();
    for (int64_t kk = c0 / 2 + w; kk < c1 / 2; kk += nw) {
        const int r = a.rels[a.si[kk]];
        T vr[2];
        lane_pair_load(bf.rel + (int64_t)r * ld, n, vr);
        const double* pp = run_l + (kk * 2 - c0) * 2 * n;
        double ep = 0, en = 0;
#pragma unroll
        for (int k = 0; k < 2; ++k) {
            const int i = 2 * l + k;
            if (i >= n) continue;
            const double dp = pp[n + i] - pp[i] - (double)vr[k];
            const double dn = pp[3 * n + i] - pp[2 * n + i] - (double)vr[k];
            ep += a.l1 ? fabs(dp) : dp * dp;
            en += a.l1 ? fabs(dn) : dn * dn;
        }
        ep = wave_sum(ep);
        en = wave_sum(en);
        const bool active = ep + a.margin > en;
        if (l == 0) {
            a.act[kk] = active ? 1 : 0;
            a.loss[kk] = active ? a.margin + ep - en : 0.0;
            act_l[kk - c0 / 2] = active;
        }
    }
    ptab_clear_next(a, (int64_t)blockIdx.x * blockDim.x + threadIdx.x, (int64_t)gridDim.x * blockDim.x);
    __syncthreads();
    if (pent >= 0 && act_l[threadIdx.x >> 2])
        ptab_insert(a, prel, pent, (int)(c0 / 2) * 4 + (int)threadIdx.x);
}


static __attribute__((unused)) __global__ __launch_bounds__(256) void rtile_count_kernel(const uint64_t* keys, const int32_t* seg_start,
                                                          const int32_t* nseg_p, int64_t cap, KeyLayout kl,
                                                          int32_t ne, int32_t St, int32_t* ntiles,
                                                          int32_t* rel_begin) {
    const int nseg = *nseg_p;
    for (int64_t s = (int64_t)blockIdx.x * blockDim.x + threadIdx.x; s < cap; s += (int64_t)gridDim.x * blockDim.x) {
        if (s >= nseg) {
            ntiles[s] = 0;
            continue;
        }
        const uint64_t k = keys[seg_start[s]];
        const int row = kl.row_of(k);
        const bool isrel = row >= ne;
        const int ns = (seg_start[s + 1] - seg_start[s]) / 2;
        ntiles[s] = isrel ? (ns + St - 1) / St : 0;
        if (isrel) {
            const bool first = s == 0 || kl.batch_of(keys[seg_start[s - 1]]) != kl.batch_of(k) ||
                               kl.row_of(keys[seg_start[s - 1]]) < ne;
            if (first) rel_begin[kl.batch_of(k)] = (int32_t)s;
        }
    }
}

static __attribute__((unused)) __global__ __launch_bounds__(256) void rtile_scatter_kernel(const int32_t* ntiles, const int32_t* tile_first,
                                                            const int32_t* nseg_p, RTile* tiles) {
    const int nseg = *nseg_p;
    for (int s = blockIdx.x * blockDim.x + threadIdx.x; s < nseg; s += gridDim.x * blockDim.x)
        for (int q = 0; q < ntiles[s]; ++q) tiles[tile_first[s] + q] = RTile{s, q};
}

struct RTileDescArgs {
    const uint64_t* keys;
    const int32_t* seg_start;
    const int32_t* seg_row;
    const RTile* tiles;
    const int32_t* tile_first;
    const int32_t* nseg;
    const int32_t* batch_seg;
    int32_t nb, St, ne, B;
    int32_t sub, Bs;
    KeyLayout kl;
    const int32_t* si;
    const int32_t* sj;
    const uint8_t* side;
    const int32_t* heads;
    const int32_t* tails;
    int32_t* batch_t0;
    int32_t* td_r;
    int32_t* td_cnt;
    int32_t* td_kk;
    int32_t* td_ent;
};

static __attribute__((unused)) __global__ __launch_bounds__(256) void rtile_desc_kernel(RTileDescArgs a) {
    const int ntiles = a.tile_first[*a.nseg];
    const int gid = blockIdx.x * blockDim.x + threadIdx.x;
    if (gid <= a.nb) a.batch_t0[gid] = a.tile_first[a.batch_seg[gid]];
    for (int64_t x = gid; x < (int64_t)ntiles * 8; x += (int64_t)gridDim.x * blockDim.x) {
        const int t = (int)(x >> 3), q = (int)(x & 7);
        const RTile tl = a.tiles[t];
        const int p0 = a.seg_start[tl.seg], p1 = a.seg_start[tl.seg + 1];
        const int f = tl.q * a.St, cnt = min(a.St, (p1 - p0) / 2 - f);
        if (q == 0) {
            a.td_r[t] = a.seg_row[tl.seg] - a.ne;
            const bool single = a.tile_first[tl.seg + 1] - a.tile_first[tl.seg] == 1;
            a.td_cnt[t] = cnt | (single ? 256 : 0);
        }
        int kk = 0, e4[4] = {-1, -1, -1, -1};
        if (q < cnt) {
            const uint64_t key = a.keys[p0 + 2 * (f + q)];
            kk = a.kl.kk_of(key);
            const int ib = a.kl.batch_of(key);
            const int64_t k = (int64_t)(ib / a.sub) * a.B + (int64_t)(ib % a.sub) * a.Bs + kk;
            const int i0 = a.si[k], jj = a.sj[k];
            const int h = a.heads[i0], tt = a.tails[i0];
            const bool sd = a.side[k] != 0;
            e4[0] = h;
            e4[1] = tt;
            e4[2] = sd ? h : jj;
            e4[3] = sd ? jj : tt;
        }
        a.td_kk[x] = kk;
        *(int4*)(a.td_ent + 4 * x) = make_int4(e4[0], e4[1], e4[2], e4[3]);
    }
}

}
```

kb2e_amd/csrc/kernels_transr_wave.hpp:

```cpp
#pragma once

#include "kernels_transr_cons.hpp"

namespace kb2e {

template <int Q>
__device__ __forceinline__ float quad_bcast(float x) {
    return __int_as_float(__builtin_amdgcn_mov_dpp(__float_as_int(x), Q * 0x55, 0xF, 0xF, false));
}
template <int Q>
__device__ __forceinline__ double quad_bcast(double x) {
    const long long b = __double_as_longlong(x);
    const int lo = __builtin_amdgcn_mov_dpp((int)(b & 0xffffffff), Q * 0x55, 0xF, 0xF, false);
    const int hi = __builtin_amdgcn_mov_dpp((int)(b >> 32), Q * 0x55, 0xF, 0xF, false);
    return __longlong_as_double(((long long)hi << 32) | (unsigned)lo);
}

constexpr int kProjWaves = 2;

template <typename T>
__host__ __device__ constexpr int proj_wave_rows(int KS) {
    return sizeof(T) == 8 ? 4 * KS : 16 * ((KS + 3) / 4);
}

template <typename T, int KS>
__global__ __launch_bounds__(128) void transr_proj_wave_kernel(RParArgs a, RParBufs<T> bf) {
    using M = Mfma16<T>;
    constexpr int NB = (KS + 3) / 4, NP = 16 * NB, L = NP + 2, NS = NP / 4, R = proj_wave_rows<T>(KS);
    extern __shared__ __attribute__((aligned(16))) char smem[];
    if (!a.compat) ptab_clear_next(a, (int64_t)blockIdx.x * blockDim.x + threadIdx.x, (int64_t)gridDim.x * blockDim.x);
    const int t = a.batch_t0[a.batch] + blockIdx.x;
    if (t >= a.batch_t0[a.batch + 1]) return;
    const int r = a.td_r[t], cnt = a.td_cnt[t] & 255;
    const int n = a.n, ld = a.ld;
    const int w = threadIdx.x >> 6, l = lane_id(), kq = l >> 4, l16 = l & 15;
    T* Wl = (T*)smem;
    const int q = w * 4 + (l16 >> 2), which = l16 & 3;
    const bool has = q < cnt;
    const int kk = a.td_kk[t * 8 + q];
    const int ed = a.td_ent[(t * 8 + q) * 4 + which];
    const int e = ed < 0 ? 0 : ed;
    {
        using T2 = typename std::conditional<sizeof(T) == 8, double2, float2>::type;
        constexpr int kPairs = R * L / 2, kThreads = kProjWaves * kWave;
        constexpr int kPer = (kPairs + kThreads - 1) / kThreads;
        const T2* Wg = (const T2*)(bf.W + (int64_t)r * n * ld);
        const int hp = ld / 2;
        T2 v[kPer];
#pragma unroll
        for (int p = 0; p < kPer; ++p) {
            const int idx = threadIdx.x + p * kThreads;
            const int j = idx / (L / 2), ip = idx % (L / 2);
            const bool ok = idx < kPairs && j < n && ip < hp;
            const T2 g = Wg[ok ? j * hp + ip : 0];
            v[p] = ok ? g : T2{T(0), T(0)};
        }
#pragma unroll
        for (int p = 0; p < kPer; ++p) {
            const int idx = threadIdx.x + p * kThreads;
            if (idx < kPairs) ((T2*)Wl)[idx] = v[p];
        }
    }
    T vf[KS], rf[KS];
    {
        const T* vr = bf.ent + (int64_t)e * ld;
        const T* rr = bf.rel + (int64_t)r * ld;
#pragma unroll
        for (int s = 0; s < KS; ++s) {
            const int k = kmap<T>(s, kq);
            const T m = (has && k < n) ? T(1) : T(0);
            vf[s] = vr[k < n ? k : 0] * m;
            rf[s] = rr[k < n ? k : 0] * m;
        }
    }
    __syncthreads();
    if (w * 16 >= 4 * cnt) return;
    T pf[NS];
#pragma unroll
    for (int ib = 0; ib < NB; ++ib) {
        typename M::acc_t acc = {T(0), T(0), T(0), T(0)};
#pragma unroll
        for (int s = 0; s < KS; ++s) acc = M::mma(Wl[kmap<T>(s, kq) * L + ib * 16 + l16], vf[s], acc);
#pragma unroll
        for (int k = 0; k < 4; ++k) pf[4 * ib + k] = acc[k];
    }
    const bool upd = has && (which & 1);
    const int u = which >> 1;
    T xf[NS];
    T en = T(0);
    T* xrow = bf.x + ((int64_t)kk * 2 + u) * ld;
    T* drow = bf.d + ((int64_t)kk * 2 + u) * ld;
    double* prow = a.proj + ((int64_t)kk * 4 + which) * ld;
#pragma unroll
    for (int s = 0; s < NS; ++s) xf[s] = T(0);
#pragma unroll
    for (int s = 0; s < KS; ++s) {
        const int k = kmap<T>(s, kq);
        const T ph = (which & 2) ? quad_bcast<2>(pf[s]) : quad_bcast<0>(pf[s]);
        const T vh = (which & 2) ? quad_bcast<2>(vf[s]) : quad_bcast<0>(vf[s]);
        const T dp = pf[s] - ph - rf[s];
        en += a.l1 ? fabs(dp) : dp * dp;
        xf[s] = upd && k < n ? (a.l1 ? (dp > T(0) ? T(1) : T(-1)) : T(2) * dp) : T(0);
        if (upd && k < n) {
            xrow[k] = xf[s];
            drow[k] = vh - vf[s];
        }
        if (a.compat && has && k < n) prow[k] = (double)pf[s];
    }
    if (!a.compat) {
        const T er = row4_sum(en);
        const T ep = quad_bcast<1>(er);
        if (has && which == 3 && kq == 0) {
            const bool active = (double)ep + a.margin > (double)er;
            a.act[kk] = active ? 1 : 0;
            a.loss[kk] = active ? a.margin + (double)ep - (double)er : 0.0;
        }
        const T en3 = quad_bcast<3>(er);
        if (has && kq == 0 && (double)ep + a.margin > (double)en3) ptab_insert(a, r, e, kk * 4 + which);
    }
    T* yrow = bf.y + ((int64_t)kk * 2 + u) * ld;
#pragma unroll
    for (int jb = 0; jb < NB; ++jb) {
        typename M::acc_t acc = {T(0), T(0), T(0), T(0)};
#pragma unroll
        for (int s = 0; s < KS; ++s) {
            const int jr = jb * 16 + l16;
            acc = M::mma(jr < R ? Wl[jr * L + kmap<T>(s, kq)] : T(0), xf[s], acc);
        }
#pragma unroll
        for (int k = 0; k < 4; ++k) {
            const int j = jb * 16 + M::row(l, k);
            if (upd && j < n) yrow[j] = acc[k];
        }
    }
}

template <typename T, int KS>
__global__ __launch_bounds__(256) void transr_grad_wave_kernel(RParArgs a, RParBufs<T> bf) {
    using M = Mfma16<T>;
    constexpr int NB = (KS + 3) / 4;
    constexpr int kOut = (NB * NB + kConsWaves - 1) / kConsWaves;
    constexpr int kSteps = 4;
    const int t = a.batch_t0[a.batch] + blockIdx.x;
    if (t >= a.batch_t0[a.batch + 1]) return;
    const int r = a.td_r[t], cnt = a.td_cnt[t] & 255, single = (a.td_cnt[t] >> 8) & 1;
    const int n = a.n, ld = a.ld;
    const int w = threadIdx.x >> 6, l = lane_id(), kq = l >> 4, l16 = l & 15;
    const int nu = 2 * cnt;
    int rowu[kSteps];
    T cu[kSteps];
#pragma unroll
    for (int s = 0; s < kSteps; ++s) {
        const int u = 4 * s + kq;
        const int kk = a.td_kk[t * 8 + (u >> 1)], side = u & 1;
        rowu[s] = kk * 2 + side;
        cu[s] = (u < nu && a.act[kk]) ? (T)(-(side ? 1.0 : -1.0) * a.lr) : T(0);
    }
    T* const wp = bf.wpart + (int64_t)blockIdx.x * n * ld;
#pragma unroll
    for (int q = 0; q < kOut; ++q) {
        const int tile = w + kConsWaves * q;
        if (tile >= NB * NB) break;
        const int jb = tile / NB, ib = tile % NB;
        const int j = jb * 16 + l16, i = ib * 16 + l16;
        T av[kSteps], bv[kSteps];
#pragma unroll
        for (int s = 0; s < kSteps; ++s) {
            av[s] = cu[s] * bf.d[(int64_t)rowu[s] * ld + (j < n ? j : 0)] * (j < n ? T(1) : T(0));
            bv[s] = bf.x[(int64_t)rowu[s] * ld + (i < n ? i : 0)] * (i < n ? T(1) : T(0));
        }
        typename M::acc_t acc = {T(0), T(0), T(0), T(0)};
#pragma unroll
        for (int s = 0; s < kSteps; ++s) acc = M::mma(av[s], bv[s], acc);
#pragma unroll
        for (int k = 0; k < 4; ++k) {
            const int jj = jb * 16 + M::row(l, k);
            if (jj < n && i < n) wp[(int64_t)jj * ld + i] = acc[k];
        }
        if (jb == 0) {
            typename M::acc_t dr = {T(0), T(0), T(0), T(0)};
#pragma unroll
            for (int s = 0; s < kSteps; ++s) dr = M::mma(l16 == 0 ? cu[s] : T(0), bv[s], dr);
            if (M::row(l, 0) == 0 && i < n) bf.rpart[(int64_t)blockIdx.x * ld + i] = dr[0];
        }
    }
    if (w == 0) {
        const bool au = l < nu && a.act[a.td_kk[t * 8 + (l >> 1)]] != 0;
        const uint64_t m = __ballot(au);
        if (l == 0) a.tile_act[t] = __builtin_popcountll(m);
    }
    if (w == kConsWaves - 1) {
        __shared__ int ents[kCPairs];
        const RTile tl = a.tiles[t];
        bool relpair = false;
        if (tl.q == 0 && r < a.ne) {
            const int p0 = a.seg_start[tl.seg], ns = (a.seg_start[tl.seg + 1] - p0) / 2;
            for (int m0 = 0; m0 < ns && !relpair; m0 += kWave)
                relpair = __ballot(m0 + l < ns && a.act[a.kl.kk_of(a.keys[p0 + 2 * (m0 + l)])]) != 0;
        }
        const int pq = l;
        int ent = -1, slot = -1;
        if (pq < 4 * cnt) {
            const int q = pq >> 2, u = (pq >> 1) & 1, role = pq & 1;
            const int kk = a.td_kk[t * 8 + q];
            if (a.act[kk]) {
                slot = (kk * 2 + u) * 2 + role;
                const int e = a.td_ent[t * 32 + pq];
                if (!transr_pair_dup(a, slot, r, e)) ent = e;
            }
        } else if (pq == 4 * cnt && relpair && !transr_relpair_dup(a, r)) {
            ent = r;
            slot = -2;
        }
        ents[pq] = ent;
        wave_lds_sync();
        bool dup = false;
        for (int k = 0; k < kCPairs; k += 4) {
            const int4 e4 = *(const int4*)(ents + k);
            dup |= (k < pq && e4.x == ent) | (k + 1 < pq && e4.y == ent) | (k + 2 < pq && e4.z == ent) |
                   (k + 3 < pq && e4.w == ent);
        }
        const bool live = ent >= 0 && !dup;
        const uint64_t m = __ballot(live);
        const int pos = __builtin_popcountll(m & ((1ull << l) - 1));
        int32_t* cp = bf.cpairs + (int64_t)blockIdx.x * 2 * kCPairs;
        if (live) {
            cp[pos] = ent;
            cp[kCPairs + pos] = slot;
        } else if (slot >= 0) {
            bf.pflag[slot] = 0;
        }
        if (l == 0) bf.cnrows[blockIdx.x] = __builtin_popcountll(m) | (single << 7) | (r << 8);
    }
}

}
```

kb2e_amd/csrc/transr_cons.hip:

```cpp
#include "transr_cons.hpp"

#include <algorithm>
#include <cstring>
#include <stdexcept>
#include <string>
#include <utility>

#include "hip_util.hpp"
#include "kernels_transr_cons.hpp"
#include "kernels_transr_seq.hpp"
#include "kernels_transr_chainw.hpp"
#include "kernels_transr_chainwp.hpp"
#include "kernels_transr_chaing.hpp"
#include "kernels_transr_pipe.hpp"
#include "kernels_transr_wave.hpp"

namespace kb2e {

namespace {

enum Kind { kCons, kGrad, kProj };

int chain_grid(const RParArgs& a) { return a.nrel > 0 ? a.nrel : 1; }

template <typename T, int KS>
const void* fn_at(Kind k) {
    return k == kCons ? (const void*)transr_cons_wave_kernel<T, KS>
           : k == kGrad ? (const void*)transr_grad_wave_kernel<T, KS>
                        : (const void*)transr_proj_wave_kernel<T, KS>;
}

template <typename T, int... KS>
const void* fn_table(Kind k, int ks, std::integer_sequence<int, KS...>) {
    const void* tab[] = {fn_at<T, KS + 1>(k)...};
    return tab[ks - 1];
}

template <typename T>
const void* kernel_fn(Kind k, int n) {
    if (!cons_wave_supported(n)) throw std::runtime_error("TransR wave kernels: n > 64");
    return fn_table<T>(k, cons_live_steps<T>(n), std::make_integer_sequence<int, 16>{});
}

template <typename T>
const void* cons_fn(int n) {
    return kernel_fn<T>(kCons, n);
}

template <bool STATS, int... KS>
const void* pipe_table(int ks, std::integer_sequence<int, KS...>) {
    const void* tab[] = {(const void*)transr_cons_pipe_kernel<double, KS + 1, STATS>...};
    return tab[ks - 1];
}

const void* pipe_fn(int n, bool stats) {
    if (!cons_wave_supported(n)) throw std::runtime_error("transRNorm pipelined chain kernel: n > 64");
    const auto seq = std::make_integer_sequence<int, 16>{};
    return stats ? pipe_table<true>((n + 3) / 4, seq) : pipe_table<false>((n + 3) / 4, seq);
}

const void* chainw_fn(int n) {
    switch (wide_nb(n)) {
        case 1: return (const void*)transr_cons_chain_wide_kernel<1>;
        case 2: return (const void*)transr_cons_chain_wide_kernel<2>;
        case 3: return (const void*)transr_cons_chain_wide_kernel<3>;
        case 4: return (const void*)transr_cons_chain_wide_kernel<4>;
        case 5: return (const void*)transr_cons_chain_wide_kernel<5>;
        case 6: return (const void*)transr_cons_chain_wide_kernel<6>;
        case 7: return (const void*)transr_cons_chain_wide_kernel<7>;
    }
    throw std::runtime_error("transRNorm wide chain kernel: n > 112");
}

const void* chainwp_fn(int n) {
    switch (wp_ks(n)) {
        case 18: return (const void*)transr_cons_chain_wpipe_kernel<18>;
        case 20: return (const void*)transr_cons_chain_wpipe_kernel<20>;
        case 22: return (const void*)transr_cons_chain_wpipe_kernel<22>;
        case 24: return (const void*)transr_cons_chain_wpipe_kernel<24>;
        case 25: return (const void*)transr_cons_chain_wpipe_kernel<25>;
    }
    throw std::runtime_error("transRNorm pipelined wide chain kernel: no instantiation");
}

bool use_wpipe(int n) {
    const char* e = getenv("KB2E_RPAR_CHAIN");
    return n > 64 && n <= kWPMaxN && !(e && std::string(e) == "lockstep");
}

}

size_t cons_seq_setup(int n) {
    const size_t lds = pipe_lds<double>(n);
    for (const bool stats : {false, true})
        HIPCHK(hipFuncSetAttribute(pipe_fn(n, stats), hipFuncAttributeMaxDynamicSharedMemorySize, (int)lds));
    return lds;
}

void cons_seq_launch(const RParArgs& a, const RParBufs<double>& bf, size_t lds, hipStream_t stream) {
    RParArgs aa = a;
    RParBufs<double> bb = bf;
    void* args[] = {&aa, &bb};
    HIPCHK(hipLaunchKernel(pipe_fn(a.n, bf.stats != 0), dim3(chain_grid(a)), dim3(kChainThreads), args, lds, stream));
}

bool cons_chainw_supported(int n) { return n >= 1 && n <= kWideMaxN; }

size_t cons_chainw_setup(int n) {
    HIPCHK(hipFuncSetAttribute((const void*)transr_cons_da_rel_kernel, hipFuncAttributeMaxDynamicSharedMemorySize,
                               (int)da_rel_lds(n)));
    const bool wp = use_wpipe(n);
    const size_t lds = wp ? chainwp_lds(n) : chainw_lds(n);
    HIPCHK(hipFuncSetAttribute(wp ? chainwp_fn(n) : chainw_fn(n), hipFuncAttributeMaxDynamicSharedMemorySize,
                               (int)lds));
    return lds;
}

bool cons_chainw_pipelined(int n) { return use_wpipe(n); }

void cons_chainw_launch(const RParArgs& a, const RParBufs<double>& bf, size_t lds, hipStream_t stream) {
    RParArgs aa = a;
    RParBufs<double> bb = bf;
    void* args[] = {&aa, &bb};
    const int grid = chain_grid(a);
    if (use_wpipe(a.n)) {
        HIPCHK(hipLaunchKernel(chainwp_fn(a.n), dim3(grid), dim3(kWPThreads), args, lds, stream));
    } else {
        HIPCHK(hipLaunchKernel(chainw_fn(a.n), dim3(grid), dim3(kWideThreads), args, lds, stream));
        HIPCHK(hipLaunchKernel((const void*)transr_cons_da_rel_kernel, dim3(grid), dim3(kDaRelThreads), args,
                               da_rel_lds(a.n), stream));
    }
}

bool cons_wave_supported(int n) { return n >= 1 && n <= 64; }

size_t cons_wave_setup(int n, int St, int esize) {
    const size_t lds = esize == 8 ? rcons_lds<double>(n, St) : rcons_lds<float>(n, St);
    HIPCHK(hipFuncSetAttribute(esize == 8 ? cons_fn<double>(n) : cons_fn<float>(n),
                               hipFuncAttributeMaxDynamicSharedMemorySize, (int)lds));
    return lds;
}

template <typename T>
void cons_wave_launch(const RParArgs& a, const RParBufs<T>& bf, int grid, size_t lds, hipStream_t stream) {
    RParArgs aa = a;
    RParBufs<T> bb = bf;
    void* args[] = {&aa, &bb};
    HIPCHK(hipLaunchKernel(cons_fn<T>(a.n), dim3(grid), dim3(kConsWaves * kWave), args, lds, stream));
}

template <typename T>
void grad_wave_launch(const RParArgs& a, const RParBufs<T>& bf, int grid, hipStream_t stream) {
    RParArgs aa = a;
    RParBufs<T> bb = bf;
    void* args[] = {&aa, &bb};
    HIPCHK(hipLaunchKernel(kernel_fn<T>(kGrad, a.n), dim3(grid), dim3(kConsWaves * kWave), args, 0, stream));
}

template <typename T>
void proj_wave_launch(const RParArgs& a, const RParBufs<T>& bf, int grid, hipStream_t stream) {
    RParArgs aa = a;
    RParBufs<T> bb = bf;
    void* args[] = {&aa, &bb};
    const size_t lds = sizeof(T) * (size_t)proj_wave_rows<T>(cons_live_steps<T>(a.n)) * rm_ld(a.n);
    HIPCHK(hipLaunchKernel(kernel_fn<T>(kProj, a.n), dim3(grid), dim3(kProjWaves * kWave), args, lds, stream));
}

bool cons_chaing_supported(int n) { return n >= 1 && n <= kGenMaxN; }

size_t cons_chaing_setup(int n, int esize) {
    const size_t lds = chaing_lds(n);
    HIPCHK(hipFuncSetAttribute(esize == 8 ? (const void*)transr_cons_chain_gen_kernel<double>
                                          : (const void*)transr_cons_chain_gen_kernel<float>,
                               hipFuncAttributeMaxDynamicSharedMemorySize, (int)lds));
    return lds;
}

template <typename T>
void cons_chaing_launch(const RParArgs& a, const RParBufs<T>& bf, size_t lds, hipStream_t stream) {
    RParArgs aa = a;
    RParBufs<T> bb = bf;
    void* args[] = {&aa, &bb};
    HIPCHK(hipLaunchKernel((const void*)transr_cons_chain_gen_kernel<T>, dim3(chain_grid(a)), dim3(kGenThreads), args,
                           lds, stream));
}
template void cons_chaing_launch<double>(const RParArgs&, const RParBufs<double>&, size_t, hipStream_t);
template void cons_chaing_launch<float>(const RParArgs&, const RParBufs<float>&, size_t, hipStream_t);

template void proj_wave_launch<double>(const RParArgs&, const RParBufs<double>&, int, hipStream_t);
template void proj_wave_launch<float>(const RParArgs&, const RParBufs<float>&, int, hipStream_t);

template void grad_wave_launch<double>(const RParArgs&, const RParBufs<double>&, int, hipStream_t);
template void grad_wave_launch<float>(const RParArgs&, const RParBufs<float>&, int, hipStream_t);

template void cons_wave_launch<double>(const RParArgs&, const RParBufs<double>&, int, size_t, hipStream_t);
template void cons_wave_launch<float>(const RParArgs&, const RParBufs<float>&, int, size_t, hipStream_t);

void cons_seq_take_stats(unsigned long long (&st)[64]) {
    HIPCHK(hipMemcpyFromSymbol(st, HIP_SYMBOL(g_seq_stats), sizeof(st)));
    unsigned long long z[64] = {};
    HIPCHK(hipMemcpyToSymbol(HIP_SYMBOL(g_seq_stats), z, sizeof(z)));
}

void cons_wave_take_stats(unsigned long long (&st)[16]) {
    unsigned long long mine[16];
    HIPCHK(hipMemcpyFromSymbol(mine, HIP_SYMBOL(g_cons_stats), sizeof(mine)));
    for (int k = 0; k < 16; ++k) st[k] = (k == 2 || k == 6) ? std::max(st[k], mine[k]) : st[k] + mine[k];
    std::memset(mine, 0, sizeof(mine));
    HIPCHK(hipMemcpyToSymbol(HIP_SYMBOL(g_cons_stats), mine, sizeof(mine)));
}

}
```

kb2e_amd/csrc/transr_cons.hpp:

```cpp
#pragma once

#include <hip/hip_runtime.h>

#include "kernels_transr_parallel.hpp"

namespace kb2e {

constexpr int kWideMaxN = 112;
constexpr int kConsPpt = 1;

bool cons_wave_supported(int n);
size_t cons_wave_setup(int n, int St, int esize);
template <typename T>
void cons_wave_launch(const RParArgs& a, const RParBufs<T>& bf, int grid, size_t lds, hipStream_t stream);
template <typename T>
void proj_wave_launch(const RParArgs& a, const RParBufs<T>& bf, int grid, hipStream_t stream);
template <typename T>
void grad_wave_launch(const RParArgs& a, const RParBufs<T>& bf, int grid, hipStream_t stream);
size_t cons_seq_setup(int n);
void cons_seq_launch(const RParArgs& a, const RParBufs<double>& bf, size_t lds, hipStream_t stream);
bool cons_chainw_supported(int n);
size_t cons_chainw_setup(int n);
void cons_chainw_launch(const RParArgs& a, const RParBufs<double>& bf, size_t lds, hipStream_t stream);
bool cons_chaing_supported(int n);
size_t cons_chaing_setup(int n, int esize);
template <typename T>
void cons_chaing_launch(const RParArgs& a, const RParBufs<T>& bf, size_t lds, hipStream_t stream);
bool cons_chainw_pipelined(int n);
void cons_seq_take_stats(unsigned long long (&st)[64]);
void cons_wave_take_stats(unsigned long long (&st)[16]);

constexpr int kWideParMaxN = 512;
struct WideGeom {
    int St = 1;
    int chunk = 2;
    size_t tile_lds = 0, scan_lds = 0, chain_lds = 0;
};
bool wide_par_supported(int n);
WideGeom wide_setup(int n, int ld, int esize);
template <typename T>
void wide_phase_a(const RParArgs& a, const RParBufs<T>& bf, const WideGeom& g, int tgrid, double* scan,
                  double* scan_pre, const double* work_in, double* work_out, hipStream_t st);
template <typename T>
void wide_phase_b(const RParArgs& a, const RParBufs<T>& bf, const WideGeom& g, double* wsc, bool constraint,
                  int rel_segs_max, hipStream_t st);

}
```

Baseline: 9.065 million.

## Merge phase A of all TransR sub-batches into single batched kernel launches

When a batch is split into sub-batches on the MFMA wave path, the projection, scan-energy and gradient (phase A) kernels for all sub-batches now run as single launches. Each block maps to its sub-batch through a view offset. The per-sub-batch parameter snapshots and double-buffered side stream are dropped in this mode, and only the apply/constraint phase B runs per sub-batch. This cuts launch count and snapshot copies, but phase A for later sub-batches now reads parameters from before the earlier sub-batches' updates rather than a snapshot, and the tile and ptab buffers grow per sub-batch.

Result: faster. 9.414 million (median of 6 runs) (+3.9%).

```diff
diff --git a/kb2e_amd/csrc/engine.hip b/kb2e_amd/csrc/engine.hip
--- a/kb2e_amd/csrc/engine.hip
+++ b/kb2e_amd/csrc/engine.hip
@@ -164,6 +164,9 @@
     DevBuf rpar_y, rpar_wpart, rpar_rpart, rpar_tile_act, rpar_pair, rpar_relpair, rpar_relpair_stamp, rpar_scan_pre, rpar_tiles,
         rpar_ntiles, rpar_tile_first, rpar_rel_begin, rpar_scan;
     DevBuf rpar_ptab;
+    bool rpar_merge_a = false;
+    RParMerge rpar_merge{};
+    uint32_t rpar_merge_batches = 0;
     DevBuf rpar_batch_t0, rpar_td_r, rpar_td_cnt, rpar_td_kk, rpar_td_ent;
     DevBuf sh_rpar_batch_t0, sh_rpar_td_r, sh_rpar_td_cnt, sh_rpar_td_kk, sh_rpar_td_ent;
     DevBuf rpar_brel, sh_rpar_brel, rpar_bnrel, sh_rpar_bnrel;
diff --git a/kb2e_amd/csrc/engine_transr_parallel.inc b/kb2e_amd/csrc/engine_transr_parallel.inc
--- a/kb2e_amd/csrc/engine_transr_parallel.inc
+++ b/kb2e_amd/csrc/engine_transr_parallel.inc
@@ -89,8 +89,28 @@
     const int64_t nkeys = c->S * c->slots;
     c->rpar_y.alloc((size_t)c->B * 2 * c->ld * es);
     const bool cw = cons_wave_supported(c->n) && mst > 0;
-    c->rpar_wpart.alloc((size_t)c->rpar_max_tiles * (cw ? kConsPpt : 1) * c->n * c->ld * es);
-    c->rpar_rpart.alloc((size_t)c->rpar_max_tiles * c->ld * es);
+    c->rpar_merge_a = false;
+    c->rpar_merge = RParMerge{};
+    if (c->sub > 1 && c->rpar_mfma && cw && c->rpar_St <= 8 && !(ck0 && std::string(ck0) == "tile")) {
+        const char* ma = getenv("KB2E_RPAR_MERGE_A");
+        const char* sp = getenv("KB2E_RPAR_SCAN_PREFIX");
+        const int64_t nch = (2 * c->Bs + kScanChunk - 1) / kScanChunk;
+        const bool use_pre = g.transr_compat && (sp ? sp[0] == '1' : nch > kScanDirectMax);
+        c->rpar_merge_a = !(ma && ma[0] == '0') && !use_pre;
+    }
+    int64_t tslots = c->rpar_max_tiles;
+    if (c->rpar_merge_a) {
+        RParMerge& m = c->rpar_merge;
+        m.sub = c->sub;
+        m.Bs = (int32_t)c->Bs;
+        m.Blast = (int32_t)(c->B - (int64_t)(c->sub - 1) * c->Bs);
+        m.tcap = (int32_t)(std::min<int64_t>(g.num_relations, c->Bs) + c->Bs / c->rpar_St + 1);
+        m.nch = (int32_t)((2 * c->Bs + kScanChunk - 1) / kScanChunk);
+        m.brel_cap = (int32_t)std::min<int64_t>(g.num_relations, c->Bs);
+        tslots = (int64_t)m.sub * m.tcap;
+    }
+    c->rpar_wpart.alloc((size_t)tslots * (cw ? kConsPpt : 1) * c->n * c->ld * es);
+    c->rpar_rpart.alloc((size_t)tslots * c->ld * es);
     c->rpar_tile_act.alloc((size_t)(nkeys + 1) * 4);
     c->rpar_pair.alloc((size_t)c->B * 4 * c->ld * es);
     c->rpar_relpair.alloc((size_t)g.num_relations * c->ld * es);
@@ -111,7 +131,7 @@
     }
     if (c->rpar_widep) c->rpar_wsc.alloc((size_t)c->rpar_brel_cap * c->n * c->ld * 8);
     else c->rpar_wsc.free();
-    if (c->sub > 1) {
+    if (c->sub > 1 && !c->rpar_merge_a) {
         c->snap_ent.alloc(c->ent.bytes);
         c->snap_rel.alloc(c->rel.bytes);
         c->snap_w.alloc(c->w.bytes);
@@ -131,20 +151,24 @@
         throw std::invalid_argument("PARALLEL TransR: at most 2^24 - 2 entities, 2^18 - 2 relations, 2^20 - 1 samples a batch");
     {
         size_t sz = 1024;
-        while (sz < (size_t)c->B * 4 * 3) sz <<= 1;
+        while (sz < (size_t)(c->rpar_merge_a ? c->Bs : c->B) * 4 * 3) sz <<= 1;
+        const size_t ntab = c->rpar_merge_a ? 2 * (size_t)c->sub : 3;
         c->rpar_ptab_mask = (uint32_t)(sz - 1);
-        c->rpar_ptab.alloc(3 * sz * 8);
-        memset_sync(c->rpar_ptab.p, 0xff, 3 * sz * 8);
+        c->rpar_ptab.alloc(ntab * sz * 8);
+        memset_sync(c->rpar_ptab.p, 0xff, ntab * sz * 8);
+        c->rpar_merge_batches = 0;
     }
     const int scan_chunk = c->rpar_widep ? c->rpar_wg.chunk : kScanChunk;
-    c->rpar_scan.alloc((size_t)((2 * c->B + scan_chunk - 1) / scan_chunk) * 2 * c->n * 8);
+    c->rpar_scan.alloc((size_t)std::max<int64_t>((2 * c->B + scan_chunk - 1) / scan_chunk,
+                                                  (int64_t)c->rpar_merge.sub * c->rpar_merge.nch) *
+                       2 * c->n * 8);
     c->rpar_scan_pre.alloc(c->rpar_scan.bytes);
     c->rpar_pflag.alloc((size_t)c->B * 4);
-    c->rpar_cons_tile.alloc((size_t)c->rpar_max_tiles * (cw ? kConsPpt : 1) * 4);
+    c->rpar_cons_tile.alloc((size_t)tslots * (cw ? kConsPpt : 1) * 4);
     if (cw) {
-        c->rpar_cpairs.alloc((size_t)c->rpar_max_tiles * 2 * kCPairs * 4);
-        c->rpar_vio.alloc((size_t)c->rpar_max_tiles * kCPairs * 4);
-        c->rpar_cnrows.alloc((size_t)c->rpar_max_tiles * 4);
+        c->rpar_cpairs.alloc((size_t)tslots * 2 * kCPairs * 4);
+        c->rpar_vio.alloc((size_t)tslots * kCPairs * 4);
+        c->rpar_cnrows.alloc((size_t)tslots * 4);
     }
     size_t tb = 0;
     HIPCHK(hipcub::DeviceScan::ExclusiveSum(nullptr, tb, (int32_t*)nullptr, (int32_t*)nullptr, (int)(nkeys + 1),
@@ -180,6 +204,7 @@
                                           hipFuncAttributeMaxDynamicSharedMemorySize, (int)l2);
         const char* ck = getenv("KB2E_RPAR_CONS");
         c->rpar_cons_wave = cw && c->rpar_St <= 8 && !(ck && std::string(ck) == "tile");
+        if (c->rpar_merge_a && !c->rpar_cons_wave) throw std::logic_error("merged phase A off the wave path");
         if (c->rpar_cons_wave) c->rpar_cons_lds = cons_wave_setup(c->n, c->rpar_St, c->esize);
         c->rpar_cons_seq = c->rpar_cons_wave && c->f64() && !(ck && std::string(ck) == "jacobi");
         if (c->rpar_cons_seq) {
@@ -218,13 +243,15 @@
             {&c->sb_cpairs, &c->rpar_cpairs}, {&c->sb_vio, &c->rpar_vio}, {&c->sb_cnrows, &c->rpar_cnrows}};
         for (const auto& pr : sets) {
             pr.first->free();
-            if (c->sub > 1 && pr.second->p) {
+            if (c->sub > 1 && !c->rpar_merge_a && pr.second->p) {
                 pr.first->alloc(pr.second->bytes);
                 memset_sync(pr.first->p, 0, pr.first->bytes);
             }
         }
     }
-    for (const void* k : {(const void*)rpar_scan_energy_kernel<double>, (const void*)rpar_scan_energy_kernel<float>})
+    for (const void* k : {(const void*)rpar_scan_energy_kernel<double>, (const void*)rpar_scan_energy_kernel<float>,
+                          (const void*)rpar_scan_energy_merged_kernel<double>,
+                          (const void*)rpar_scan_energy_merged_kernel<float>})
         (void)hipFuncSetAttribute(k, hipFuncAttributeMaxDynamicSharedMemorySize, (int)rpar_scan_lds(c));
     (void)hipGetLastError();
 }
@@ -291,15 +318,11 @@
 }
 
 template <typename T>
-void run_subbatch_transr_parallel(kb2e_ctx* c, int64_t b, int j) {
-    const bool ov = c->sub > 1 && sub_overlap_on();
-    const bool side = ov && j > 0;
-    const int set = ov ? (j & 1) : 0;
-    hipStream_t sa = side ? c->suba_stream : c->stream;
+void fill_rpar(kb2e_ctx* c, int64_t b, int j, int set, RParArgs& a, RParBufs<T>& bf) {
     const int64_t ib = b * c->sub + j;
     const int64_t first = b * c->B + (int64_t)j * c->Bs;
     const int64_t cnt = std::min<int64_t>(c->Bs, c->B - (int64_t)j * c->Bs);
-    RParArgs a{};
+    a = RParArgs{};
     a.heads = c->heads.as<int32_t>();
     a.tails = c->tails.as<int32_t>();
     a.rels = c->rels.as<int32_t>();
@@ -338,14 +361,7 @@
     a.brel = c->rpar_brel.as<int32_t>() + ib * c->rpar_brel_cap;
     a.nrel = c->pin_bnrel[ib];
     if (a.nrel < 1 || a.nrel > c->rpar_brel_cap) throw std::logic_error("batch relation count out of range");
-    {
-        unsigned long long* t0 = c->rpar_ptab.as<unsigned long long>();
-        const size_t sz = (size_t)c->rpar_ptab_mask + 1;
-        a.ptab = t0 + (c->batch_stamp % 3) * sz;
-        a.ptab_next = t0 + ((c->batch_stamp + 1) % 3) * sz;
-        a.ptab_mask = c->rpar_ptab_mask;
-    }
-    RParBufs<T> bf{};
+    bf = RParBufs<T>{};
     bf.ent = c->ent.as<T>();
     bf.rel = c->rel.as<T>();
     bf.W = c->w.as<T>();
@@ -357,7 +373,6 @@
     bf.pair = c->rpar_pair.as<T>();
     bf.relpair = c->rpar_relpair.as<T>();
     bf.relpair_stamp = c->rpar_relpair_stamp.as<uint32_t>();
-    bf.stamp = ++c->batch_stamp;
     bf.err = c->dataflow_err.as<uint32_t>() + 1;
     if (c->rpar_mfma) {
         bf.pflag = buf_set(set, c->rpar_pflag, c->sb_pflag).as<uint8_t>();
@@ -379,6 +394,28 @@
         bf.stats = getenv("KB2E_RPAR_STATS") != nullptr;
         bf.last_renorm = 1;
     }
+}
+
+template <typename T>
+void transr_phase_b(kb2e_ctx* c, RParArgs a, RParBufs<T> bf);
+
+template <typename T>
+void run_subbatch_transr_parallel(kb2e_ctx* c, int64_t b, int j) {
+    const bool ov = c->sub > 1 && sub_overlap_on();
+    const bool side = ov && j > 0;
+    const int set = ov ? (j & 1) : 0;
+    hipStream_t sa = side ? c->suba_stream : c->stream;
+    RParArgs a;
+    RParBufs<T> bf;
+    fill_rpar<T>(c, b, j, set, a, bf);
+    {
+        unsigned long long* t0 = c->rpar_ptab.as<unsigned long long>();
+        const size_t sz = (size_t)c->rpar_ptab_mask + 1;
+        a.ptab = t0 + (c->batch_stamp % 3) * sz;
+        a.ptab_next = t0 + ((c->batch_stamp + 1) % 3) * sz;
+        a.ptab_mask = c->rpar_ptab_mask;
+    }
+    bf.stamp = ++c->batch_stamp;
     RParBufs<T> bfa = bf;
     if (c->sub > 1) {
         bfa.ent = c->snap_ent.as<T>();
@@ -413,12 +450,8 @@
     }
     const size_t lds = rpar_lds<T>(c);
     const int tgrid = c->rpar_max_tiles;
-    const int rel_waves = (int)std::min<int64_t>(c->cfg.num_relations, c->B) * (c->n + 1);
-    const int rgrid = (rel_waves + 3) / 4;
-    const int egrid = 256;
     const bool mf = c->rpar_mfma;
     const size_t lt = mf ? rmfma_lds<T>(c, false) : lds;
-    const size_t lc = mf ? rmfma_lds<T>(c, true) : lds;
     const int tb = mf ? c->rpar_tile_threads : 256;
     auto tile = [&](auto proj, auto grad) {
         constexpr bool P = decltype(proj)::value, G = decltype(grad)::value;
@@ -475,6 +508,19 @@
         }
     });
     a_done();
+    transr_phase_b<T>(c, a, bf);
+    b_done();
+    if (c->pending.size() > 4096) c->flush_timers();
+}
+
+template <typename T>
+void transr_phase_b(kb2e_ctx* c, RParArgs a, RParBufs<T> bf) {
+    const int tgrid = c->rpar_merge_a ? c->rpar_merge.tcap : c->rpar_max_tiles;
+    const int rel_waves = (int)std::min<int64_t>(c->cfg.num_relations, c->B) * (c->n + 1);
+    const int rgrid = (rel_waves + 3) / 4;
+    const int egrid = 256;
+    const bool mf = c->rpar_mfma;
+    const size_t lc = mf ? rmfma_lds<T>(c, true) : rpar_lds<T>(c);
     hipEvent_t e0, e1;
     c->ev_begin("apply", e0);
     const char* fz = getenv("KB2E_RPAR_FUSE");
@@ -494,7 +540,6 @@
     if (c->rpar_no_constraint) {
         c->ev_end(e1);
         c->launch(rows_fn(yes1()), dim3(fgrid), dim3(1024), 0, e0, e1, a, bf, kRParLongMin, egrid);
-        b_done();
         return;
     }
     if (fuse) {
@@ -532,12 +577,54 @@
         HIPCHK(hipGetLastError());
         c->launch(transr_entity_kernel<T, false>, dim3(egrid), dim3(1024), 0, nullptr, e1, a, bf, kRParLongMin);
     }
-    b_done();
+}
+
+template <typename T>
+void run_batch_transr_merged(kb2e_ctx* c, int64_t b) {
+    const RParMerge& m = c->rpar_merge;
+    RParArgs a0;
+    RParBufs<T> bf0;
+    fill_rpar<T>(c, b, 0, 0, a0, bf0);
+    {
+        unsigned long long* t0 = c->rpar_ptab.as<unsigned long long>();
+        const size_t gsz = (size_t)m.sub * ((size_t)c->rpar_ptab_mask + 1);
+        const uint32_t grp = c->rpar_merge_batches++ & 1;
+        a0.ptab = t0 + grp * gsz;
+        a0.ptab_next = t0 + (grp ^ 1) * gsz;
+        a0.ptab_mask = c->rpar_ptab_mask;
+    }
+    c->timed("score", [&] {
+        proj_wave_merged_launch<T>(a0, bf0, m, c->stream);
+        if (c->cfg.transr_compat) {
+            const int last = (int)((2 * (int64_t)m.Blast + kScanChunk - 1) / kScanChunk);
+            const int grid = (m.sub - 1) * m.nch + last;
+            rpar_scan_sums_merged_kernel<<<grid, 256, 0, c->stream>>>(a0.proj, m, c->ld, c->n,
+                                                                         c->rpar_scan.as<double>());
+            rpar_scan_energy_merged_kernel<T><<<grid, 1024, rpar_scan_lds(c), c->stream>>>(
+                a0, bf0, m, c->rpar_scan.as<double>(), c->transr_work.as<double>(), c->transr_work_alt.as<double>());
+            HIPCHK(hipGetLastError());
+            std::swap(c->transr_work.p, c->transr_work_alt.p);
+        }
+        grad_wave_merged_launch<T>(a0, bf0, m, c->stream);
+    });
+    for (int j = 0; j < m.sub; ++j) {
+        RParArgs a = a0;
+        RParBufs<T> bf = bf0;
+        rpar_sub_view(a, bf, m, j);
+        a.nrel = c->pin_bnrel[b * c->sub + j];
+        if (a.nrel < 1 || a.nrel > c->rpar_brel_cap) throw std::logic_error("batch relation count out of range");
+        bf.stamp = ++c->batch_stamp;
+        transr_phase_b<T>(c, a, bf);
+    }
     if (c->pending.size() > 4096) c->flush_timers();
 }
 
 template <typename T>
 void run_batch_transr_parallel(kb2e_ctx* c, int64_t b) {
+    if (c->rpar_merge_a) {
+        run_batch_transr_merged<T>(c, b);
+        return;
+    }
     if (c->sub > 1) {
         for (auto pr : {std::make_pair(&c->snap_ent, &c->ent), std::make_pair(&c->snap_rel, &c->rel),
                         std::make_pair(&c->snap_w, &c->w)})
diff --git a/kb2e_amd/csrc/kernels_transr_parallel.hpp b/kb2e_amd/csrc/kernels_transr_parallel.hpp
--- a/kb2e_amd/csrc/kernels_transr_parallel.hpp
+++ b/kb2e_amd/csrc/kernels_transr_parallel.hpp
@@ -173,6 +173,50 @@
 
 __host__ __device__ constexpr int rm_up16_host_dev(int v) { return (v + 15) & ~15; }
 constexpr int kCPairs = 64;
+
+struct RParMerge {
+    int32_t sub;
+    int32_t Bs;
+    int32_t Blast;
+    int32_t tcap;
+    int32_t nch;
+    int32_t brel_cap;
+};
+
+template <typename P>
+__host__ __device__ __forceinline__ void rpar_advance(P*& p, int64_t k) {
+    if (p) p += k;
+}
+
+template <typename T>
+__host__ __device__ __forceinline__ void rpar_sub_view(RParArgs& a, RParBufs<T>& bf, const RParMerge& m, int j) {
+    const int64_t s0 = (int64_t)j * m.Bs, t0 = (int64_t)j * m.tcap;
+    a.B = j == m.sub - 1 ? m.Blast : m.Bs;
+    a.batch += j;
+    rpar_advance(a.si, s0);
+    rpar_advance(a.sj, s0);
+    rpar_advance(a.side, s0);
+    rpar_advance(a.act, s0);
+    rpar_advance(a.loss, s0);
+    rpar_advance(a.proj, s0 * 4 * a.ld);
+    rpar_advance(a.brel, (int64_t)j * m.brel_cap);
+    rpar_advance(a.ptab, (int64_t)j * ((int64_t)a.ptab_mask + 1));
+    rpar_advance(bf.x, s0 * 2 * a.ld);
+    rpar_advance(bf.d, s0 * 2 * a.ld);
+    rpar_advance(bf.y, s0 * 2 * a.ld);
+    rpar_advance(bf.pflag, s0 * 4);
+    rpar_advance(bf.wpart, t0 * bf.cons_ppt * a.n * a.ld);
+    rpar_advance(bf.rpart, t0 * a.ld);
+    rpar_advance(bf.cons_tile, t0 * bf.cons_ppt);
+    rpar_advance(bf.cpairs, t0 * 2 * kCPairs);
+    rpar_advance(bf.vio, t0 * kCPairs);
+    rpar_advance(bf.cnrows, t0);
+}
+
+__device__ __forceinline__ void ptab_clear_group(const RParArgs& a, int sub, int64_t tid, int64_t nthreads) {
+    const int64_t words = (int64_t)sub * ((int64_t)a.ptab_mask + 1);
+    for (int64_t q = tid; q < words; q += nthreads) a.ptab_next[q] = kPtabEmpty;
+}
 
 template <typename T>
 __host__ __device__ constexpr int rpar_lds_w(int n, int ld) {
@@ -872,9 +916,8 @@
 
 constexpr int kScanChunk = 64;
 
-static __attribute__((unused)) __global__ __launch_bounds__(256) void rpar_scan_sums_kernel(const double* proj, int64_t calls, int32_t ld,
-                                                             int32_t n, double* sums) {
-    const int c = blockIdx.x;
+__device__ __forceinline__ void rpar_scan_sums_block(const double* proj, int64_t calls, int32_t ld, int32_t n,
+                                                     double* sums, int c) {
     const int64_t c0 = (int64_t)c * kScanChunk, c1 = min<int64_t>(calls, c0 + kScanChunk);
     for (int e = threadIdx.x; e < 2 * n; e += blockDim.x) {
         const int side = e / n, i = e % n;
@@ -888,6 +931,18 @@
         }
         sums[(int64_t)c * 2 * n + e] = (s[0] + s[1]) + (s[2] + s[3]);
     }
+}
+
+static __attribute__((unused)) __global__ __launch_bounds__(256) void rpar_scan_sums_kernel(const double* proj, int64_t calls, int32_t ld,
+                                                             int32_t n, double* sums) {
+    rpar_scan_sums_block(proj, calls, ld, n, sums, blockIdx.x);
+}
+
+static __attribute__((unused)) __global__ __launch_bounds__(256) void rpar_scan_sums_merged_kernel(const double* proj, RParMerge m, int32_t ld,
+                                                                    int32_t n, double* sums) {
+    const int j = blockIdx.x / m.nch, c = blockIdx.x - j * m.nch;
+    const int64_t calls = 2 * (int64_t)(j == m.sub - 1 ? m.Blast : m.Bs);
+    rpar_scan_sums_block(proj + (int64_t)j * m.Bs * 4 * ld, calls, ld, n, sums + (int64_t)j * m.nch * 2 * n, c);
 }
 
 constexpr int kScanDirectMax = 256;
@@ -927,13 +982,49 @@
     }
 }
 
-template <typename T>
-__global__ __launch_bounds__(1024) void rpar_scan_energy_kernel(RParArgs a, RParBufs<T> bf, const double* sums,
-                                                                int32_t nchunks, const double* work_in,
-                                                                double* work_out, const double* pre) {
-    extern __shared__ __attribute__((aligned(16))) char smem[];
-    double* run_l = (double*)smem;
-    const int c = blockIdx.x, n = a.n, ld = a.ld;
+__device__ __forceinline__ void rpar_scan_parts(const double* sums, int c, int E2, int G, double* part) {
+    if ((int)threadIdx.x < G * E2) {
+        const int g = threadIdx.x / E2, e = threadIdx.x % E2;
+        double s[4] = {0, 0, 0, 0};
+        for (int q0 = g * 16; q0 < c; q0 += G * 16) {
+            double v[16];
+#pragma unroll
+            for (int q = 0; q < 16; ++q) v[q] = q0 + q < c ? sums[(int64_t)(q0 + q) * E2 + e] : 0.0;
+#pragma unroll
+            for (int q = 0; q < 16; ++q) s[q & 3] += v[q];
+        }
+        part[g * E2 + e] = (s[0] + s[1]) + (s[2] + s[3]);
+    }
+}
+__device__ __forceinline__ double rpar_scan_start(const double* work_in, const double* part, int E2, int G, int e) {
+    double p = 0.0;
+    for (int g = 0; g < G; ++g) p += part[g * E2 + e];
+    return work_in[e] + p;
+}
+template <bool KEEP>
+__device__ __forceinline__ double rpar_scan_calls(double run, const double* proj, int64_t c0, int64_t c1, int n,
+                                                  int ld, int e, double* run_l) {
+    const int side = e / n, i = e % n;
+    for (int64_t k = c0; k < c1; k += 16) {
+        double v[16];
+#pragma unroll
+        for (int q = 0; q < 16; ++q) v[q] = k + q < c1 ? proj[((k + q) * 2 + side) * ld + i] : 0.0;
+#pragma unroll
+        for (int q = 0; q < 16; ++q)
+            if (k + q < c1) {
+                run += v[q];
+                if (KEEP) run_l[(k + q - c0) * 2 * n + e] = run;
+            }
+    }
+    return run;
+}
+
+template <typename T, class Clear>
+__device__ __forceinline__ void rpar_scan_energy_block(const RParArgs& a, const RParBufs<T>& bf, const double* sums,
+                                                       int c, int32_t nchunks, const double* work_in,
+                                                       double* work_out, const double* pre, double* run_l,
+                                                       Clear clear) {
+    const int n = a.n, ld = a.ld;
     const int64_t calls = 2 * (int64_t)a.B;
     const int64_t c0 = (int64_t)c * kScanChunk, c1 = min<int64_t>(calls, c0 + kScanChunk);
     __shared__ int act_l[kScanChunk / 2];
@@ -951,41 +1042,12 @@
     }
     const int E2 = 2 * n, G = max(1, (int)blockDim.x / E2);
     double* part = run_l + kScanChunk * E2;
-    if (!pre && (int)threadIdx.x < G * E2) {
-        const int g = threadIdx.x / E2, e = threadIdx.x % E2;
-        double s[4] = {0, 0, 0, 0};
-        for (int q0 = g * 16; q0 < c; q0 += G * 16) {
-            double v[16];
-#pragma unroll
-            for (int q = 0; q < 16; ++q) v[q] = q0 + q < c ? sums[(int64_t)(q0 + q) * E2 + e] : 0.0;
-#pragma unroll
-            for (int q = 0; q < 16; ++q) s[q & 3] += v[q];
-        }
-        part[g * E2 + e] = (s[0] + s[1]) + (s[2] + s[3]);
-    }
+    if (!pre) rpar_scan_parts(sums, c, E2, G, part);
     __syncthreads();
     for (int e = threadIdx.x; e < 2 * n; e += blockDim.x) {
-        double run;
-        if (pre) {
-            run = pre[(int64_t)c * E2 + e];
-        } else {
-            double p = 0.0;
-            for (int g = 0; g < G; ++g) p += part[g * E2 + e];
-            run = work_in[e] + p;
-        }
-        const int side = e / n, i = e % n;
-        for (int64_t k = c0; k < c1; k += 16) {
-            double v[16];
-#pragma unroll
-            for (int q = 0; q < 16; ++q) v[q] = k + q < c1 ? a.proj[((k + q) * 2 + side) * ld + i] : 0.0;
-#pragma unroll
-            for (int q = 0; q < 16; ++q)
-                if (k + q < c1) {
-                    run += v[q];
-                    run_l[(k + q - c0) * 2 * n + e] = run;
-                }
-        }
-        if (c == nchunks - 1) work_out[e] = run;
+        double run = pre ? pre[(int64_t)c * E2 + e] : rpar_scan_start(work_in, part, E2, G, e);
+        run = rpar_scan_calls<true>(run, a.proj, c0, c1, n, ld, e, run_l);
+        if (work_out && c == nchunks - 1) work_out[e] = run;
     }
     __syncthreads();
     const int w = threadIdx.x >> 6, nw = blockDim.x >> 6, l = lane_id();
@@ -1013,10 +1075,63 @@
             act_l[kk - c0 / 2] = active;
         }
     }
-    ptab_clear_next(a, (int64_t)blockIdx.x * blockDim.x + threadIdx.x, (int64_t)gridDim.x * blockDim.x);
+    clear();
     __syncthreads();
     if (pent >= 0 && act_l[threadIdx.x >> 2])
         ptab_insert(a, prel, pent, (int)(c0 / 2) * 4 + (int)threadIdx.x);
+}
+
+template <typename T>
+__global__ __launch_bounds__(1024) void rpar_scan_energy_kernel(RParArgs a, RParBufs<T> bf, const double* sums,
+                                                                int32_t nchunks, const double* work_in,
+                                                                double* work_out, const double* pre) {
+    extern __shared__ __attribute__((aligned(16))) char smem[];
+    double* run_l = (double*)smem;
+    rpar_scan_energy_block<T>(a, bf, sums, blockIdx.x, nchunks, work_in, work_out, pre, run_l, [&] {
+        ptab_clear_next(a, (int64_t)blockIdx.x * blockDim.x + threadIdx.x, (int64_t)gridDim.x * blockDim.x);
+    });
+}
+
+__device__ __forceinline__ const double* rpar_scan_carry_chain(const double* proj0, const RParMerge& m, int jn, int n,
+                                                               int ld, const double* sums, const double* work_in,
+                                                               double* part, double* carry_l) {
+    const int E2 = 2 * n, G = max(1, (int)blockDim.x / E2);
+    const double* win = work_in;
+    for (int jj = 0; jj < jn; ++jj) {
+        const int cl = m.nch - 1;
+        const int64_t calls = 2 * (int64_t)m.Bs;
+        const int64_t c0 = (int64_t)cl * kScanChunk, c1 = min<int64_t>(calls, c0 + kScanChunk);
+        rpar_scan_parts(sums + (int64_t)jj * m.nch * E2, cl, E2, G, part);
+        __syncthreads();
+        double run = 0.0;
+        if ((int)threadIdx.x < E2)
+            run = rpar_scan_calls<false>(rpar_scan_start(win, part, E2, G, threadIdx.x),
+                                         proj0 + (int64_t)jj * m.Bs * 4 * ld, c0, c1, n, ld, threadIdx.x, nullptr);
+        __syncthreads();
+        if ((int)threadIdx.x < E2) carry_l[threadIdx.x] = run;
+        win = carry_l;
+    }
+    if (jn > 0) __syncthreads();
+    return win;
+}
+
+template <typename T>
+__global__ __launch_bounds__(1024) void rpar_scan_energy_merged_kernel(RParArgs a, RParBufs<T> bf, RParMerge m,
+                                                                       const double* sums, const double* work_in,
+                                                                       double* work_out) {
+    extern __shared__ __attribute__((aligned(16))) char smem[];
+    double* run_l = (double*)smem;
+    __shared__ double carry_l[128];
+    const int j = blockIdx.x / m.nch, c = blockIdx.x - j * m.nch;
+    const int n = a.n, ld = a.ld, E2 = 2 * n;
+    const double* win =
+        rpar_scan_carry_chain(a.proj, m, j, n, ld, sums, work_in, run_l + kScanChunk * E2, carry_l);
+    rpar_sub_view(a, bf, m, j);
+    const int nchunks = (int)((2 * (int64_t)a.B + kScanChunk - 1) / kScanChunk);
+    rpar_scan_energy_block<T>(a, bf, sums + (int64_t)j * m.nch * E2, c, nchunks, win,
+                              j == m.sub - 1 ? work_out : nullptr, nullptr, run_l, [&] {
+        ptab_clear_group(a, m.sub, (int64_t)blockIdx.x * blockDim.x + threadIdx.x, (int64_t)gridDim.x * blockDim.x);
+    });
 }
 
 
diff --git a/kb2e_amd/csrc/kernels_transr_wave.hpp b/kb2e_amd/csrc/kernels_transr_wave.hpp
--- a/kb2e_amd/csrc/kernels_transr_wave.hpp
+++ b/kb2e_amd/csrc/kernels_transr_wave.hpp
@@ -24,12 +24,11 @@
 }
 
 template <typename T, int KS>
-__global__ __launch_bounds__(128) void transr_proj_wave_kernel(RParArgs a, RParBufs<T> bf) {
+__device__ __forceinline__ void transr_proj_wave_block(const RParArgs& a, const RParBufs<T>& bf, int bid) {
     using M = Mfma16<T>;
     constexpr int NB = (KS + 3) / 4, NP = 16 * NB, L = NP + 2, NS = NP / 4, R = proj_wave_rows<T>(KS);
     extern __shared__ __attribute__((aligned(16))) char smem[];
-    if (!a.compat) ptab_clear_next(a, (int64_t)blockIdx.x * blockDim.x + threadIdx.x, (int64_t)gridDim.x * blockDim.x);
-    const int t = a.batch_t0[a.batch] + blockIdx.x;
+    const int t = a.batch_t0[a.batch] + bid;
     if (t >= a.batch_t0[a.batch + 1]) return;
     const int r = a.td_r[t], cnt = a.td_cnt[t] & 255;
     const int n = a.n, ld = a.ld;
@@ -136,12 +135,27 @@
 }
 
 template <typename T, int KS>
-__global__ __launch_bounds__(256) void transr_grad_wave_kernel(RParArgs a, RParBufs<T> bf) {
+__global__ __launch_bounds__(128) void transr_proj_wave_kernel(RParArgs a, RParBufs<T> bf) {
+    if (!a.compat) ptab_clear_next(a, (int64_t)blockIdx.x * blockDim.x + threadIdx.x, (int64_t)gridDim.x * blockDim.x);
+    transr_proj_wave_block<T, KS>(a, bf, blockIdx.x);
+}
+
+template <typename T, int KS>
+__global__ __launch_bounds__(128) void transr_proj_wave_merged_kernel(RParArgs a, RParBufs<T> bf, RParMerge m) {
+    if (!a.compat)
+        ptab_clear_group(a, m.sub, (int64_t)blockIdx.x * blockDim.x + threadIdx.x, (int64_t)gridDim.x * blockDim.x);
+    const int j = blockIdx.x / m.tcap;
+    rpar_sub_view(a, bf, m, j);
+    transr_proj_wave_block<T, KS>(a, bf, blockIdx.x - j * m.tcap);
+}
+
+template <typename T, int KS>
+__device__ __forceinline__ void transr_grad_wave_block(const RParArgs& a, const RParBufs<T>& bf, int bid) {
     using M = Mfma16<T>;
     constexpr int NB = (KS + 3) / 4;
     constexpr int kOut = (NB * NB + kConsWaves - 1) / kConsWaves;
     constexpr int kSteps = 4;
-    const int t = a.batch_t0[a.batch] + blockIdx.x;
+    const int t = a.batch_t0[a.batch] + bid;
     if (t >= a.batch_t0[a.batch + 1]) return;
     const int r = a.td_r[t], cnt = a.td_cnt[t] & 255, single = (a.td_cnt[t] >> 8) & 1;
     const int n = a.n, ld = a.ld;
@@ -156,7 +170,7 @@
         rowu[s] = kk * 2 + side;
         cu[s] = (u < nu && a.act[kk]) ? (T)(-(side ? 1.0 : -1.0) * a.lr) : T(0);
     }
-    T* const wp = bf.wpart + (int64_t)blockIdx.x * n * ld;
+    T* const wp = bf.wpart + (int64_t)bid * n * ld;
 #pragma unroll
     for (int q = 0; q < kOut; ++q) {
         const int tile = w + kConsWaves * q;
@@ -181,7 +195,7 @@
             typename M::acc_t dr = {T(0), T(0), T(0), T(0)};
 #pragma unroll
             for (int s = 0; s < kSteps; ++s) dr = M::mma(l16 == 0 ? cu[s] : T(0), bv[s], dr);
-            if (M::row(l, 0) == 0 && i < n) bf.rpart[(int64_t)blockIdx.x * ld + i] = dr[0];
+            if (M::row(l, 0) == 0 && i < n) bf.rpart[(int64_t)bid * ld + i] = dr[0];
         }
     }
     if (w == 0) {
@@ -223,15 +237,27 @@
         const bool live = ent >= 0 && !dup;
         const uint64_t m = __ballot(live);
         const int pos = __builtin_popcountll(m & ((1ull << l) - 1));
-        int32_t* cp = bf.cpairs + (int64_t)blockIdx.x * 2 * kCPairs;
+        int32_t* cp = bf.cpairs + (int64_t)bid * 2 * kCPairs;
         if (live) {
             cp[pos] = ent;
             cp[kCPairs + pos] = slot;
         } else if (slot >= 0) {
             bf.pflag[slot] = 0;
         }
-        if (l == 0) bf.cnrows[blockIdx.x] = __builtin_popcountll(m) | (single << 7) | (r << 8);
-    }
-}
-
-}
+        if (l == 0) bf.cnrows[bid] = __builtin_popcountll(m) | (single << 7) | (r << 8);
+    }
+}
+
+template <typename T, int KS>
+__global__ __launch_bounds__(256) void transr_grad_wave_kernel(RParArgs a, RParBufs<T> bf) {
+    transr_grad_wave_block<T, KS>(a, bf, blockIdx.x);
+}
+
+template <typename T, int KS>
+__global__ __launch_bounds__(256) void transr_grad_wave_merged_kernel(RParArgs a, RParBufs<T> bf, RParMerge m) {
+    const int j = blockIdx.x / m.tcap;
+    rpar_sub_view(a, bf, m, j);
+    transr_grad_wave_block<T, KS>(a, bf, blockIdx.x - j * m.tcap);
+}
+
+}
diff --git a/kb2e_amd/csrc/transr_cons.hip b/kb2e_amd/csrc/transr_cons.hip
--- a/kb2e_amd/csrc/transr_cons.hip
+++ b/kb2e_amd/csrc/transr_cons.hip
@@ -19,7 +19,7 @@
 
 namespace {
 
-enum Kind { kCons, kGrad, kProj };
+enum Kind { kCons, kGrad, kProj, kGradMerged, kProjMerged };
 
 int chain_grid(const RParArgs& a) { return a.nrel > 0 ? a.nrel : 1; }
 
@@ -27,7 +27,9 @@
 const void* fn_at(Kind k) {
     return k == kCons ? (const void*)transr_cons_wave_kernel<T, KS>
            : k == kGrad ? (const void*)transr_grad_wave_kernel<T, KS>
-                        : (const void*)transr_proj_wave_kernel<T, KS>;
+           : k == kProj ? (const void*)transr_proj_wave_kernel<T, KS>
+           : k == kGradMerged ? (const void*)transr_grad_wave_merged_kernel<T, KS>
+                              : (const void*)transr_proj_wave_merged_kernel<T, KS>;
 }
 
 template <typename T, int... KS>
@@ -166,6 +168,27 @@
     HIPCHK(hipLaunchKernel(kernel_fn<T>(kProj, a.n), dim3(grid), dim3(kProjWaves * kWave), args, lds, stream));
 }
 
+template <typename T>
+void proj_wave_merged_launch(const RParArgs& a, const RParBufs<T>& bf, const RParMerge& m, hipStream_t stream) {
+    RParArgs aa = a;
+    RParBufs<T> bb = bf;
+    RParMerge mm = m;
+    void* args[] = {&aa, &bb, &mm};
+    const size_t lds = sizeof(T) * (size_t)proj_wave_rows<T>(cons_live_steps<T>(a.n)) * rm_ld(a.n);
+    HIPCHK(hipLaunchKernel(kernel_fn<T>(kProjMerged, a.n), dim3(m.sub * m.tcap), dim3(kProjWaves * kWave), args, lds,
+                           stream));
+}
+
+template <typename T>
+void grad_wave_merged_launch(const RParArgs& a, const RParBufs<T>& bf, const RParMerge& m, hipStream_t stream) {
+    RParArgs aa = a;
+    RParBufs<T> bb = bf;
+    RParMerge mm = m;
+    void* args[] = {&aa, &bb, &mm};
+    HIPCHK(hipLaunchKernel(kernel_fn<T>(kGradMerged, a.n), dim3(m.sub * m.tcap), dim3(kConsWaves * kWave), args, 0,
+                           stream));
+}
+
 bool cons_chaing_supported(int n) { return n >= 1 && n <= kGenMaxN; }
 
 size_t cons_chaing_setup(int n, int esize) {
@@ -192,6 +215,11 @@
 
 template void grad_wave_launch<double>(const RParArgs&, const RParBufs<double>&, int, hipStream_t);
 template void grad_wave_launch<float>(const RParArgs&, const RParBufs<float>&, int, hipStream_t);
+
+template void proj_wave_merged_launch<double>(const RParArgs&, const RParBufs<double>&, const RParMerge&, hipStream_t);
+template void proj_wave_merged_launch<float>(const RParArgs&, const RParBufs<float>&, const RParMerge&, hipStream_t);
+template void grad_wave_merged_launch<double>(const RParArgs&, const RParBufs<double>&, const RParMerge&, hipStream_t);
+template void grad_wave_merged_launch<float>(const RParArgs&, const RParBufs<float>&, const RParMerge&, hipStream_t);
 
 template void cons_wave_launch<double>(const RParArgs&, const RParBufs<double>&, int, size_t, hipStream_t);
 template void cons_wave_launch<float>(const RParArgs&, const RParBufs<float>&, int, size_t, hipStream_t);
diff --git a/kb2e_amd/csrc/transr_cons.hpp b/kb2e_amd/csrc/transr_cons.hpp
--- a/kb2e_amd/csrc/transr_cons.hpp
+++ b/kb2e_amd/csrc/transr_cons.hpp
@@ -17,6 +17,10 @@
 void proj_wave_launch(const RParArgs& a, const RParBufs<T>& bf, int grid, hipStream_t stream);
 template <typename T>
 void grad_wave_launch(const RParArgs& a, const RParBufs<T>& bf, int grid, hipStream_t stream);
+template <typename T>
+void proj_wave_merged_launch(const RParArgs& a, const RParBufs<T>& bf, const RParMerge& m, hipStream_t stream);
+template <typename T>
+void grad_wave_merged_launch(const RParArgs& a, const RParBufs<T>& bf, const RParMerge& m, hipStream_t stream);
 size_t cons_seq_setup(int n);
 void cons_seq_launch(const RParArgs& a, const RParBufs<double>& bf, size_t lds, hipStream_t stream);
 bool cons_chainw_supported(int n);
```
